# fdrmrc/fictitious_domain_AL_preconditioners

Hardware: AMD Instinct MI355X
Metric: FGMRES iterations/sec to 1e-8 residual, 3D Stokes-immersed (AL-preconditioned) (higher is better)
Workload: dtype f64

## Files before the change

fictitious_domain_al_preconditioners_amd/_abi.py:

```python
import ctypes as C

ALFD_MAX_BLOCKS = 3

OK, E_INVALID, E_HIP, E_NO_CONVERGENCE_OUTER, E_NO_CONVERGENCE_INNER, E_BREAKDOWN, E_NOT_SETUP, \
    E_COMM, E_UNSUPPORTED = range(9)
A, BT, B, CT, C_, M, MP, A2, KIMM = range(9)
NSLOTS = 9
SLOT_BY_NAME = {"A": A, "Bt": BT, "B": B, "Ct": CT, "C": C_, "M": M, "Mp": MP, "A2": A2, "K": KIMM}
INVW, MP_LUMPED_INV = 0, 1
NDIAGS = 2
AL2, AL_STOKES, AL_STOKES_DIAG, AL_ELL_IDEAL, AL_ELL_MODIFIED, RATIONAL = range(6)
CTRL_ABS, CTRL_REDUCTION, CTRL_FIXED_ITERS = range(3)
PREC_IDENTITY, PREC_JACOBI, PREC_CHEBYSHEV, PREC_MULTILEVEL = range(4)
INNER_OP_AUG, INNER_OP_A22, INNER_OP_AUG2 = range(3)
ORTH_MGS, ORTH_CGS, ORTH_CGS2 = range(3)
OUTER_FGMRES, OUTER_MINRES = range(2)
FGMRES_DEALII_96, FGMRES_DEALII_95 = range(2)
W_DIAGONAL, W_MASS_INV_SQUARED, W_MASS_INV = range(3)
INNER_THROW, INNER_ACCEPT = range(2)
T_SPMV_A, T_SPMV_OTHER, T_DOT, T_VEC = range(4)
T_NCLASSES = 4
UNIQUE_ID_BYTES = 128


class Control(C.Structure):
    _fields_ = [("kind", C.c_int32), ("max_steps", C.c_int32), ("tol", C.c_double), ("reduce", C.c_double)]

    def __init__(self, kind=CTRL_ABS, max_steps=100, tol=1e-10, reduce=0.0):
        super().__init__(kind, max_steps, tol, reduce)


class Config(C.Structure):
    _fields_ = [
        ("variant", C.c_int32), ("restart", C.c_int32), ("orthogonalization", C.c_int32),
        ("grad_div_in_A", C.c_int32),
        ("gamma", C.c_double), ("gamma_grad_div", C.c_double), ("gamma2", C.c_double),
        ("outer", Control), ("inner", Control), ("mp_inner", Control),
        ("inner_prec", C.c_int32), ("cheb_degree", C.c_int32), ("cheb_power_its", C.c_int32),
        ("on_inner_failure", C.c_int32),
        ("cheb_eig_ratio", C.c_double), ("cheb_safety", C.c_double),
        ("log_level", C.c_int32), ("outer_solver", C.c_int32),
        ("rho_bound", C.c_double), ("rational", Control),
        ("ml_smooth_degree", C.c_int32), ("ml_coarse_degree", C.c_int32),
        ("ml_smooth_ratio", C.c_double), ("ml_coarse_ratio", C.c_double),
        ("aug_assembled", C.c_int32), ("w_inverse", C.c_int32),
        ("mass", Control),
        ("fgmres_flavour", C.c_int32), ("ml_smooth_degree_coarse", C.c_int32),
        ("ml_patch_degree", C.c_int32), ("ml_coarse_direct", C.c_int32), ("ml_patch_ratio", C.c_double),
    ]


class Result(C.Structure):
    _fields_ = [
        ("status", C.c_int32), ("outer_iterations", C.c_int32),
        ("initial_residual", C.c_double), ("last_residual", C.c_double),
        ("inner_iterations", C.c_int64), ("mp_iterations", C.c_int64),
        ("inner_failures", C.c_int32), ("precond_applications", C.c_int32),
        ("solve_seconds", C.c_double), ("lambda_max", C.c_double),
        ("rational_iterations", C.c_int64), ("mass_iterations", C.c_int64),
    ]

    def as_dict(self):
        return {k: getattr(self, k) for k, _ in self._fields_}


class MatrixInfo(C.Structure):
    _fields_ = [
        ("lanes", C.c_int32), ("windowed", C.c_int32), ("value_indexed", C.c_int32), ("batch_major", C.c_int32),
        ("nnz", C.c_int64), ("window_blocks", C.c_int64), ("window_fallback_blocks", C.c_int64),
        ("value_indexed_blocks", C.c_int64), ("value_indexed_nnz", C.c_int64),
        ("dictionary_entries", C.c_int64), ("value_wide_nnz", C.c_int64),
        ("algorithmic_bytes", C.c_double), ("streamed_bytes", C.c_double),
        ("shared_nnz", C.c_int64), ("batch_major_blocks", C.c_int64), ("batch_major_wide", C.c_int64),
        ("batch_major_interior_blocks", C.c_int64),
    ]


class WindowPlanInfo(C.Structure):
    _fields_ = [
        ("windowed", C.c_int32), ("value_indexed", C.c_int32), ("row_block", C.c_int32), ("max_window", C.c_int32),
        ("blocks", C.c_int64), ("fallback_blocks", C.c_int64), ("segments", C.c_int64),
        ("value_indexed_blocks", C.c_int64), ("value_indexed_nnz", C.c_int64), ("value_wide_nnz", C.c_int64),
        ("dictionary_entries", C.c_int64), ("batches", C.c_int64), ("decode_mismatches", C.c_int64),
    ]


class StreamPlanInfo(C.Structure):
    _fields_ = [
        ("ok", C.c_int32), ("max_window", C.c_int32), ("max_rows", C.c_int32), ("max_batches", C.c_int32),
        ("blocks", C.c_int64), ("batches", C.c_int64), ("segments", C.c_int64), ("dictionary_entries", C.c_int64),
        ("stream_bytes", C.c_int64), ("decode_mismatches", C.c_int64), ("rows_covered", C.c_int64),
        ("shared_nnz", C.c_int64),
    ]


def default_config(variant=AL_STOKES) -> Config:
    c = Config()
    c.variant = variant
    c.restart = 50 if variant in (AL_ELL_IDEAL, AL_ELL_MODIFIED) else 30
    c.orthogonalization = ORTH_CGS2
    c.grad_div_in_A = 1
    c.gamma, c.gamma_grad_div, c.gamma2 = 10.0, 10.0, 1e-2
    c.outer = Control(CTRL_REDUCTION, 1000, 1e-8, 1e-12)
    c.inner = Control(CTRL_ABS, 100, 1e-2, 0.0)
# ... 34 lines not shown
```

fictitious_domain_al_preconditioners_amd/csrc/alfd.hip:

```cpp

#include <hip/hip_runtime.h>
#include <rccl/rccl.h>

#include <algorithm>
#include <atomic>
#include <chrono>
#include <cmath>
#include <cstdio>
#include <cstdlib>
#include <cstring>
#include <memory>
#include <climits>
#include <condition_variable>
#include <functional>
#include <mutex>
#include <string>
#include <thread>
#include <unordered_set>
#include <vector>

#include "alfd/alfd.h"
#include "kernels.hpp"
#include "kernels_vs.hpp"

// ... 129 lines not shown
    if (v <= c.tol) return SUCCESS;
    if (step >= c.max_steps || std::isnan(v)) return FAILURE;
    return ITERATE;
  }
};

struct TimedLaunch {
  int cls;
  hipEvent_t a, b;
};

}

using namespace alfd;

struct alfd_ctx {
  int device = 0;
  hipStream_t stream = nullptr;
  hipStream_t xstream = nullptr;
  hipEvent_t ev_x = nullptr, ev_halo = nullptr;
  int overlap_halo = -1;
  std::string err;
  int rank = 0, nranks = 1;
  ncclComm_t nccl = nullptr;
  struct alfd_local_group *local = nullptr;
  alfd_host_allgather_fn host_allgather = nullptr;
  alfd_host_alltoallv_fn host_alltoallv = nullptr;
  void *host_user = nullptr;
  std::vector<char> host_send, host_recv;
  std::vector<std::vector<int64_t>> part;
  int nblocks = 0;
  int64_t n[ALFD_MAX_BLOCKS] = {0, 0, 0};
  int64_t off[ALFD_MAX_BLOCKS + 1] = {0, 0, 0, 0};
  int64_t nmax = 0;
  int64_t diag_cap = 0;
  DevCsr mat[ALFD_NSLOTS + 1];
  double *diag[ALFD_NDIAGS] = {nullptr, nullptr};
  int64_t diag_n[ALFD_NDIAGS] = {0, 0};
  alfd_config cfg;
  bool configured = false, is_setup = false;
  double *sc = nullptr;
  double *sc_host = nullptr;
  double *partial = nullptr;
  int64_t pstride = 0;
  double *gather = nullptr;
  double *dinv_aug = nullptr, *dA = nullptr, *s_aug = nullptr;
  double *dinv_a22 = nullptr, *dinv_aug2 = nullptr;
  double lam_max[7] = {0, 0, 0, 0, 0, 0, 0};
  double *dinv_k = nullptr;
  double *dinv_m = nullptr, *m_tmp = nullptr, *m_tmp2 = nullptr;
  double *n_r = nullptr, *n_z = nullptr, *n_p = nullptr, *n_Ap = nullptr;
  double *n_sc = nullptr, *n_sc_host = nullptr, *n_partial = nullptr, *n_gather = nullptr;
  int64_t mass_its = 0;
  int n_owner = 0;
  double *gd_bx = nullptr, *gd_q = nullptr;
  int nmp_group = 16;
  int nmp_host_stepped = 0;
  HostCsr h_M, h_K;
  std::vector<int32_t> ml_agg[ALFD_MAX_LEVELS];
  std::vector<double> ml_wgt[ALFD_MAX_LEVELS];
  int64_t ml_ncoarse[ALFD_MAX_LEVELS] = {0, 0, 0, 0, 0, 0, 0, 0};
  HostCsr ml_P[ALFD_MAX_LEVELS];
  DevCsr ml_inv;
  struct Patch {
    bool on = false;
    int64_t m = 0, mpad = 0;
    DevCsr Ass, As, Ats, Cs, Cts;
    int32_t *S = nullptr;
    double *dinv = nullptr, *rS = nullptr, *zS = nullptr, *uS = nullptr, *eS = nullptr, *cd = nullptr,
           *cres = nullptr, *ctmp = nullptr, *rr = nullptr;
    double lmax = 0;
    uint8_t *tail_mask = nullptr;
    bool rep = false;
    int64_t m_loc = 0, piece = 1, lam_piece = 1;
    std::vector<int64_t> soff;
    DevCsr Cts_loc, Ctg;
    double *send = nullptr, *stage = nullptr, *lam_send = nullptr, *lam_stage = nullptr, *loc = nullptr;
  } patch;
  std::vector<MlLevel> ml;
  int ml_rep_level = -1;
  bool dots_replicated = false;
  int64_t ml_rep_threshold = 300000;
  int ml_fuse = 1;
  int ml_gpu_galerkin = 1;
  double *g_w = nullptr, *g_tlam = nullptr;
  std::vector<int64_t> ml_coff[ALFD_MAX_LEVELS];
  const int64_t *up_col_offsets = nullptr;
  bool up_local_only = false;
  DevCsr rat_mat;
  double *rt_r = nullptr, *rt_z = nullptr, *rt_p = nullptr, *rt_Ap = nullptr, *rt_x = nullptr;
  double *rt_dinv = nullptr, *rt_partial = nullptr, *rt_scb = nullptr, *rt_coef = nullptr;
  double *rt_scb_host = nullptr;
  int64_t rational_its = 0;
  int64_t wmax = 0;
  std::vector<void *> ws_allocs;
  double *w_r = nullptr, *w_z = nullptr, *w_p = nullptr, *w_Ap = nullptr;
  double *c_d = nullptr, *c_res = nullptr, *c_tmp = nullptr;
  double *t_lam = nullptr;
  double *q_tmp = nullptr, *rhs_tmp = nullptr;
  double *V = nullptr, *Z = nullptr, *xb = nullptr, *bb = nullptr, *io = nullptr;
  double *st_in = nullptr, *st_out = nullptr;
  double lambda_max = 0, lambda_min = 0;
  int64_t inner_its = 0, mp_its = 0;
  int inner_failures = 0, precond_applications = 0;
  std::vector<double> history;
  int timing = 0;
  std::vector<TimedLaunch> timed;
  double t_ms[ALFD_T_NCLASSES] = {0, 0, 0, 0};
  int64_t t_launches[ALFD_T_NCLASSES] = {0, 0, 0, 0};
  double t_bytes[ALFD_T_NCLASSES] = {0, 0, 0, 0};
  double t_fbytes[ALFD_T_NCLASSES] = {0, 0, 0, 0};
  double setup_s[ALFD_SETUP_NPHASES] = {0, 0, 0, 0, 0, 0, 0, 0};
  bool upload_since_setup = false;
  std::vector<void *> allocs;
  int spmv_stream_R = 2, spmv_stream_U = 8, spmv_nt = 0, spmv_grid_mult = 8;
  int spmv_group_R = 4, spmv_group_U = 4;
  bool vi_off = false;
  int vi_rows_R = 4, vi_rows_J = 2;
  int vi_xcd = 0;
  int vi_levels = 1;
  int vi_batched = 1;
  int win_RB_vi = 96;
  int win_vi = 1;
  int win_short_scale = 2;
  int vs_enable = 1, vs_NW = 4, vs_RB = 96, vs_xcd = 0, vs_share = 1, vs_wide = 1;
  int vs_lds_base_ok = -1;
  std::vector<int64_t> rb_ptr[ALFD_NSLOTS + 1];
  std::vector<int32_t> rb_rows[ALFD_NSLOTS + 1];
  int win_short_min_blocks = 256;
  int win_min_blocks = 256;
  int win_enable = 1, win_RB = 96, win_maxW = 4096, win_gap = 8, win_xcd = 0;
  int64_t ntot() const { return off[nblocks]; }
};

struct alfd_local_group {
  int n = 0;
  std::mutex mu;
  std::condition_variable cv;
  int arrived = 0;
  long generation = 0;
  std::vector<const void *> buf;
  std::vector<const int64_t *> off;
  void barrier() {
    std::unique_lock<std::mutex> lk(mu);
    const long g = generation;
    if (++arrived == n) {
      arrived = 0;
      ++generation;
      cv.notify_all();
    } else {
      cv.wait(lk, [&] { return generation != g; });
    }
  }
};

namespace alfd {

static int comm_allgather(alfd_ctx *ctx, const void *send, void *recv, size_t bytes) {
  if (ctx->local) {
    alfd_local_group *g = ctx->local;
    HIPC(hipStreamSynchronize(ctx->stream));
    g->buf[ctx->rank] = send;
    g->barrier();
    for (int p = 0; p < g->n; ++p)
      HIPC(hipMemcpyAsync((char *)recv + (size_t)p * bytes, g->buf[p], bytes, hipMemcpyDeviceToDevice,
                          ctx->stream));
// ... 259 lines not shown
    else ALFD_WIN(3, 0);
  } else {
    if (epi == 0) ALFD_WIN(0, 1);
    else if (epi == 1) ALFD_WIN(1, 1);
    else if (epi == 2) ALFD_WIN(2, 1);
    else ALFD_WIN(3, 1);
  }
#undef ALFD_WIN
}

template <int L, int R, int U>
static void launch_window_group(alfd_ctx *ctx, const DevCsr &m, const double *x, double *y, int epi,
                                double alpha, const double *d, double *y2) {
  const size_t lds = (size_t)m.win_maxW * sizeof(double);
#define ALFD_WING(EPI, TAG)                                                                               \
  hipLaunchKernelGGL((spmv_window_group_kernel<L, R, U, EPI, TAG>), dim3((unsigned)m.win_nblocks),       \
                     dim3(kBlock), lds, ctx->stream, m.nrows, m.win_RB, m.rp, m.col, m.lcol, m.val,        \
                     m.blk_seg_begin, m.blk_W, m.seg_col, m.seg_off, x, m.halo, m.n_local_cols, y, alpha, \
                     d, y2)
  if (m.tag == 0) {
    if (epi == 0) ALFD_WING(0, 0);
    else if (epi == 1) ALFD_WING(1, 0);
    else if (epi == 2) ALFD_WING(2, 0);
    else ALFD_WING(3, 0);
  } else {
    if (epi == 0) ALFD_WING(0, 1);
    else if (epi == 1) ALFD_WING(1, 1);
    else if (epi == 2) ALFD_WING(2, 1);
    else ALFD_WING(3, 1);
  }
#undef ALFD_WING
}

template <int L>
static bool launch_window_group_RU(alfd_ctx *ctx, const DevCsr &m, const double *x, double *y, int epi,
                                   double alpha, const double *d, double *y2) {
  const int R = ctx->spmv_group_R, U = ctx->spmv_group_U;
#define ALFD_RU(RR, UU) \
  if (R == RR && U == UU) return launch_window_group<L, RR, UU>(ctx, m, x, y, epi, alpha, d, y2), true
  ALFD_RU(4, 4); ALFD_RU(2, 4); ALFD_RU(4, 2); ALFD_RU(8, 4); ALFD_RU(8, 2);
#undef ALFD_RU
  return false;
}

static bool launch_window_RU(alfd_ctx *ctx, const DevCsr &m, const double *x, double *y, int epi,
                             double alpha, const double *d, double *y2) {
  if (m.L == 32) return launch_window_group_RU<32>(ctx, m, x, y, epi, alpha, d, y2);
  if (m.L == 16) return launch_window_group_RU<16>(ctx, m, x, y, epi, alpha, d, y2);
  if (m.L == 8) return launch_window_group_RU<8>(ctx, m, x, y, epi, alpha, d, y2);
  if (m.L != 64) return false;
  const int R = ctx->spmv_stream_R, U = ctx->spmv_stream_U;
#define ALFD_RU(RR, UU) \
  if (R == RR && U == UU) return launch_window<RR, UU>(ctx, m, x, y, epi, alpha, d, y2), true
  ALFD_RU(1, 4); ALFD_RU(2, 4); ALFD_RU(2, 8); ALFD_RU(4, 2); ALFD_RU(4, 4); ALFD_RU(4, 8); ALFD_RU(8, 4);
  ALFD_RU(1, 8); ALFD_RU(1, 16); ALFD_RU(2, 16);
#undef ALFD_RU
  return false;
}


template <int L>
static void launch_vss(alfd_ctx *ctx, const DevCsr &m, const double *x, double *y, int epi, double alpha,
                       const double *d, double *y2) {
  const DevCsr::Vs &v = m.vs;
  const size_t lds = (size_t)kVsWinOff + (size_t)v.maxW * sizeof(double);
#define ALFD_VSS(EPI, TAG)                                                                                          \
  hipLaunchKernelGGL((spmv_vss_kernel<L, EPI, TAG>), dim3((unsigned)v.nb), dim3(256), lds, ctx->stream, v.stream, \
                     v.sb, v.tab, v.cnt, v.stride, v.seg_begin, v.blkW, v.seg_col, v.seg_off, v.doff, v.dn, v.dict, \
                     x, m.halo, m.n_local_cols, y, alpha, d, y2)
  if (m.tag == 0) {
    if (epi == 0) ALFD_VSS(0, 0);
    else if (epi == 1) ALFD_VSS(1, 0);
    else if (epi == 2) ALFD_VSS(2, 0);
    else ALFD_VSS(3, 0);
  } else {
    if (epi == 0) ALFD_VSS(0, 1);
    else if (epi == 1) ALFD_VSS(1, 1);
    else if (epi == 2) ALFD_VSS(2, 1);
    else ALFD_VSS(3, 1);
  }
#undef ALFD_VSS
}

static bool launch_vs(alfd_ctx *ctx, const DevCsr &m, const double *x, double *y, int epi, double alpha,
                      const double *d, double *y2, int64_t first_block = 0, int64_t n_blocks = -1) {
  const DevCsr::Vs &v = m.vs;
  if (ctx->vs_lds_base_ok < 0) {
    uint32_t *probe = nullptr, base = 1;
    if (hipMalloc((void **)&probe, sizeof(uint32_t)) == hipSuccess) {
      hipLaunchKernelGGL(vs_lds_base_probe_kernel, dim3(1), dim3(64), 4096, ctx->stream, probe);
      hipMemcpyAsync(&base, probe, sizeof(uint32_t), hipMemcpyDeviceToHost, ctx->stream);
      hipStreamSynchronize(ctx->stream);
      hipFree(probe);
    }
    ctx->vs_lds_base_ok = base == 0 ? 1 : 0;
    if (!ctx->vs_lds_base_ok)
      std::fprintf(stderr, "[alfd] dynamic LDS does not start at offset 0 (%u): batch-major SpMV formats disabled\n", base);
  }
  if (!ctx->vs_lds_base_ok) return false;
  if (v.L == 32) return launch_vss<32>(ctx, m, x, y, epi, alpha, d, y2), true;
  if (v.L == 16) return launch_vss<16>(ctx, m, x, y, epi, alpha, d, y2), true;
  if (v.L == 8) return launch_vss<8>(ctx, m, x, y, epi, alpha, d, y2), true;
  const int NW = ctx->vs_NW;
  const size_t lds = (size_t)(v.wide ? VsFmt<1>::kWinOff : VsFmt<0>::kWinOff) + (size_t)v.maxW * sizeof(double);
  if (n_blocks < 0) n_blocks = v.nb - first_block;
  if (n_blocks <= 0) return true;
  const unsigned grid = (unsigned)n_blocks;
  const int32_t base = (int32_t)first_block;
#define ALFD_VS_ARGS \
  v.stream, v.tab, v.stride, v.hdrb, v.segx, v.seg_stride, v.dict, x, m.halo, m.n_local_cols, y, alpha, d, y2, ctx->vs_xcd, base
#define ALFD_VS(EPI, NWV)                                                                                        \
  do {                                                                                                           \
    if (v.wide)                                     \
      hipLaunchKernelGGL((spmv_vs_kernel<EPI, 0, 4, 1>), dim3(grid), dim3(256), lds, ctx->stream,     \
                         ALFD_VS_ARGS);                                                                          \
    else if (m.tag == 0)                                                                                         \
      hipLaunchKernelGGL((spmv_vs_kernel<EPI, 0, NWV>), dim3(grid), dim3(64 * NWV), lds, ctx->stream, \
                         ALFD_VS_ARGS);                                                                          \
    else                \
      hipLaunchKernelGGL((spmv_vs_kernel<EPI, 1, 4>), dim3(grid), dim3(256), lds, ctx->stream,        \
                         ALFD_VS_ARGS);                                                                          \
  } while (0)
#define ALFD_VS_E(NWV)                  \
  do {                                  \
    if (epi == 0) ALFD_VS(0, NWV);      \
    else if (epi == 1) ALFD_VS(1, NWV); \
    else if (epi == 2) ALFD_VS(2, NWV); \
    else ALFD_VS(3, NWV);               \
  } while (0)
  if (NW == 8) ALFD_VS_E(8);
  else if (NW == 2) ALFD_VS_E(2);
  else ALFD_VS_E(4);
#undef ALFD_VS_E
#undef ALFD_VS
#undef ALFD_VS_ARGS
  return true;
}

static int halo_exchange(alfd_ctx *ctx, DevCsr &m, const double *x, hipStream_t st = nullptr);
static int spmv_launch_local(alfd_ctx *ctx, DevCsr &m, const double *x, double *y, int epi, double alpha, const double *d,
                             double *y2);

static int spmv_m(alfd_ctx *ctx, DevCsr &m, int cls, const double *x, double *y, int epi, double alpha = 0.0,
                  const double *d = nullptr, double *y2 = nullptr) {
  if (!m.present) return ctx->err = "matrix not set", ALFD_E_NOT_SETUP;
  const bool exchange = ctx->nranks > 1 && !m.rep && (ctx->local || ctx->host_alltoallv || m.n_halo > 0 || m.send_off.back() > 0);
  const bool overlap = exchange && (ctx->overlap_halo > 0 || (ctx->overlap_halo < 0 && (ctx->local || ctx->host_alltoallv))) && ctx->xstream && m.vs.on && m.vs.L == 64 && ctx->vs_enable && !ctx->vi_off &&
                       m.vs.nb_interior > 0 && !m.sparse && m.n_list > 0;
  if (overlap) {
    Timer tm(ctx, cls, m.algorithmic_bytes(), m.streamed_bytes(true, true));
    HIPC(hipEventRecord(ctx->ev_x, ctx->stream));
    if (!launch_vs(ctx, m, x, y, epi, alpha, d, y2, 0, m.vs.nb_interior)) return ctx->err = "batch-major launch failed", ALFD_E_HIP;
    HIPC(hipStreamWaitEvent(ctx->xstream, ctx->ev_x, 0));
    RC(halo_exchange(ctx, m, x, ctx->xstream));
    HIPC(hipEventRecord(ctx->ev_halo, ctx->xstream));
    HIPC(hipStreamWaitEvent(ctx->stream, ctx->ev_halo, 0));
    launch_vs(ctx, m, x, y, epi, alpha, d, y2, m.vs.nb_interior, m.vs.nb - m.vs.nb_interior);
    HIPC(hipGetLastError());
    return ALFD_OK;
  }
  if (exchange) RC(halo_exchange(ctx, m, x));
  if (m.sparse && epi != 1) {
    HIPC(hipMemsetAsync(y, 0, m.nrows * sizeof(double), ctx->stream));
    if (epi == 3) HIPC(hipMemsetAsync(y2, 0, m.nrows * sizeof(double), ctx->stream));
  }
  if (m.n_list == 0) return ALFD_OK;
  Timer tm(ctx, cls, m.algorithmic_bytes(), m.streamed_bytes(!ctx->vi_off, ctx->vs_enable != 0 && !ctx->vi_off));
  return spmv_launch_local(ctx, m, x, y, epi, alpha, d, y2);
}

static int spmv_launch_local(alfd_ctx *ctx, DevCsr &m, const double *x, double *y, int epi, double alpha, const double *d,
                             double *y2) {
  if (m.vs.on && ctx->vs_enable && !ctx->vi_off && launch_vs(ctx, m, x, y, epi, alpha, d, y2)) {
    HIPC(hipGetLastError());
    return ALFD_OK;
  }
  if (m.win && launch_window_RU(ctx, m, x, y, epi, alpha, d, y2)) {
    HIPC(hipGetLastError());
    return ALFD_OK;
  }
  if (m.L == 64 && !m.sparse && ctx->spmv_stream_R > 0) {
    const bool ok = ctx->spmv_nt ? launch_stream_RU<true>(ctx, m, x, y, epi, alpha, d, y2)
// ... 2569 lines not shown
  out.ncols = n_cols_c;
  out.rp.assign(1, 0);
  out.col.clear();
  out.val.clear();
  for (int t = 0; t < T; ++t) {
    for (int64_t c : t_cnt[t]) out.rp.push_back(out.rp.back() + c);
    out.col.insert(out.col.end(), t_col[t].begin(), t_col[t].end());
    out.val.insert(out.val.end(), t_val[t].begin(), t_val[t].end());
  }
}

static int upload_matrix(alfd_ctx *ctx, int slot, int64_t nrows, int64_t ncols, const int64_t *rp,
                         const int32_t *col, const double *val);
static int upload_level(alfd_ctx *ctx, DevCsr &dst, const HostCsr &h) {
  static const int32_t no_col = 0;
  static const double no_val = 0;
  RC(upload_matrix(ctx, kScratchSlot, h.nrows, h.ncols, h.rp.data(), h.col.empty() ? &no_col : h.col.data(),
                   h.val.empty() ? &no_val : h.val.data()));
  csr_free(dst);
  dst = std::move(ctx->mat[kScratchSlot]);
  ctx->mat[kScratchSlot] = DevCsr();
  dst.tag = 1;
  return ALFD_OK;
}

struct AugOp {
  DevCsr *A = nullptr, *C = nullptr, *Ct = nullptr;
  int clsA = ALFD_T_SPMV_OTHER;
  const double *w = nullptr;
  double *tlam = nullptr;
  const uint8_t *mask = nullptr;
  int64_t npad = 0;
  const double *dinv = nullptr;
  double *cd = nullptr, *cres = nullptr, *ctmp = nullptr;
  double lmax = 0;
};

struct LevelView {
  AugOp op;
  double *r = nullptr, *z = nullptr, *t = nullptr;
  DevCsr *R = nullptr, *P = nullptr;
  double *rc = nullptr, *zc = nullptr;
};

static LevelView level_view(alfd_ctx *ctx, int l) {
  MlLevel &L = ctx->ml[l];
  const bool rep = ctx->ml_rep_level >= 0 && l >= ctx->ml_rep_level;
  LevelView V;
  AugOp &F = V.op;
  F.A = rep ? &L.gA : l == 0 ? &ctx->mat[ALFD_A] : &L.A;
  F.C = rep ? &L.gC : l == 0 ? &ctx->mat[ALFD_C] : &L.C;
  F.Ct = rep ? &L.gCt : l == 0 ? &ctx->mat[ALFD_CT] : &L.Ct;
  F.clsA = l == 0 ? ALFD_T_SPMV_A : ALFD_T_SPMV_OTHER;
  F.w = rep ? ctx->g_w : ctx->diag[ALFD_INVW];
  F.tlam = rep ? ctx->g_tlam : ctx->t_lam;
  F.mask = L.tail_mask;
  F.npad = rep ? L.gnpad : L.npad;
  F.dinv = rep ? L.gdinv : L.dinv;
  F.cd = rep ? L.gcd : L.cd, F.cres = rep ? L.gcres : L.cres, F.ctmp = rep ? L.gctmp : L.ctmp;
  F.lmax = L.lmax;
  V.r = rep ? L.gr : L.r, V.z = rep ? L.gz : L.z, V.t = rep ? L.gt : L.t;
  if (l + 1 < (int)ctx->ml.size()) {
    MlLevel &N = ctx->ml[l + 1];
    V.R = rep ? &N.gR : &N.R, V.P = rep ? &N.gP : &N.P;
    V.rc = rep ? N.gr : N.r, V.zc = rep ? N.gz : N.z;
  }
  return V;
}

static AugOp patch_aug(alfd_ctx *ctx) {
  alfd_ctx::Patch &Q = ctx->patch;
  AugOp F;
  F.A = &Q.Ass, F.C = &Q.Cs, F.Ct = &Q.Cts;
  F.w = Q.rep ? ctx->g_w : ctx->diag[ALFD_INVW];
  F.tlam = Q.rep ? ctx->g_tlam : ctx->t_lam;
  F.mask = Q.tail_mask;
  F.npad = Q.mpad;
  F.dinv = Q.dinv;
  F.cd = Q.cd, F.cres = Q.cres, F.ctmp = Q.ctmp;
  F.lmax = Q.lmax;
  return F;
}

static int fused_AC(alfd_ctx *ctx, const AugOp &F, const double *x, double *y) {
  RC(spmv_m(ctx, *F.A, F.clsA, x, y, 0));
  return spmv_m(ctx, *F.C, ALFD_T_SPMV_OTHER, x, F.tlam, 2, 0.0, F.w);
}

static int aug_apply(alfd_ctx *ctx, const AugOp &F, const double *x, double *y) {
  if (ctx->cfg.aug_assembled) return spmv_m(ctx, *F.A, F.clsA, x, y, 0);
  RC(fused_AC(ctx, F, x, y));
  return spmv_m(ctx, *F.Ct, ALFD_T_SPMV_OTHER, F.tlam, y, 1, ctx->cfg.gamma);
}


static bool plain_form(const alfd_ctx *ctx, const DevCsr &m) {
  return m.present && !m.vs.on && !m.win && !(m.L == 64 && !m.sparse && ctx->spmv_stream_R > 0);
}

static bool fused_ok(const alfd_ctx *ctx, const AugOp &F) {
  return ctx->ml_fuse && ctx->nranks == 1 && !ctx->cfg.aug_assembled && !gd_nested(ctx) &&
         ctx->cfg.w_inverse == ALFD_W_DIAGONAL && F.mask && F.A->present && F.C->present && plain_form(ctx, *F.Ct);
}

static int aug_tail(alfd_ctx *ctx, const AugOp &F, int mode, const AugTailArgs &p, double vec_bytes) {
  const DevCsr &m = *F.Ct;
  const int nb_rows = m.n_list > 0 ? grid_for_rows(m.n_list, m.L) : 0;
  const unsigned grid = (unsigned)nb_rows + (unsigned)(F.npad / kChunk);
  if (grid == 0) return ALFD_OK;
  Timer tm(ctx, ALFD_T_SPMV_OTHER, m.algorithmic_bytes() + vec_bytes * (double)F.npad,
           m.streamed_bytes(false) + vec_bytes * (double)F.npad);
#define ALFD_TAIL(LL, MM)                                                                                         \
  hipLaunchKernelGGL((aug_tail_kernel<LL, MM>), dim3(grid), dim3(kBlock), 0, ctx->stream, m.n_list, m.rp, m.col,  \
                     m.val, m.sparse ? m.rows : (const int32_t *)nullptr, F.tlam, nb_rows, F.mask, p)
#define ALFD_TAIL_L(LL)                                      \
  switch (mode) {                                            \
    case TAIL_STEP: ALFD_TAIL(LL, TAIL_STEP); break;         \
    case TAIL_LAST: ALFD_TAIL(LL, TAIL_LAST); break;         \
    case TAIL_LAST_ADD: ALFD_TAIL(LL, TAIL_LAST_ADD); break; \
    case TAIL_RES: ALFD_TAIL(LL, TAIL_RES); break;           \
    case TAIL_RES_INIT: ALFD_TAIL(LL, TAIL_RES_INIT); break; \
    default: ALFD_TAIL(LL, TAIL_RES_INIT_ADD); break;        \
  }
  switch (m.L) {
    case 4: ALFD_TAIL_L(4) break;
    case 8: ALFD_TAIL_L(8) break;
    case 16: ALFD_TAIL_L(16) break;
    case 32: ALFD_TAIL_L(32) break;
    default: ALFD_TAIL_L(64) break;
  }
#undef ALFD_TAIL_L
#undef ALFD_TAIL
  HIPC(hipGetLastError());
  return ALFD_OK;
}

static int cheb_fused(alfd_ctx *ctx, const AugOp &F, int degree, double ratio, const double *r, double *z, double *zout,
                      bool have_init) {
  ChebCoef k(F.lmax, ratio);
  if (!have_init) VEC_LAUNCH(cheb_init_z_kernel, F.npad, 24, 1.0 / k.theta, F.dinv, r, z);
  for (int j = 1; j < degree; ++j) {
    RC(fused_AC(ctx, F, j == 1 ? z : F.cd, F.ctmp));
    AugTailArgs p;
    k.step(p.c1, p.c2);
    p.gamma = ctx->cfg.gamma;
    p.dinv = F.dinv, p.y = F.ctmp, p.rin = j == 1 ? r : F.cres, p.din = j == 1 ? z : F.cd;
    p.res = F.cres, p.d = F.cd, p.z = z, p.zout = zout;
    const bool last = j == degree - 1;
    RC(aug_tail(ctx, F, !last ? TAIL_STEP : zout ? TAIL_LAST_ADD : TAIL_LAST, p, last && zout ? 88.0 : 64.0));
  }
  HIPC(hipGetLastError());
  return ALFD_OK;
}

static int aug_cheb(alfd_ctx *ctx, const AugOp &F, int degree, double ratio, const double *r, double *z) {
  if (fused_ok(ctx, F)) return cheb_fused(ctx, F, degree, ratio, r, z, nullptr, false);
  return cheb_sweep(ctx, F.npad, F.dinv, F.lmax, ratio, degree, F.cd, F.cres, F.ctmp, r, z,
                    [&](const double *x, double *y) { return aug_apply(ctx, F, x, y); });
}

static int fused_residual(alfd_ctx *ctx, const AugOp &F, const double *r, double *t) {
  AugTailArgs p;
  p.gamma = ctx->cfg.gamma, p.y = t, p.rin = r, p.res = t;
  return aug_tail(ctx, F, TAIL_RES, p, 24.0);
}

static int fused_correct(alfd_ctx *ctx, const AugOp &F, int degree, double ratio, const double *r, double *t, double *zc,
                         double *zout) {
  AugTailArgs p;
// ... 56 lines not shown
  }
  if (fuse) {
    RC(fused_AC(ctx, F, z, L.t));
    RC(fused_correct(ctx, F, sdeg, c.ml_smooth_ratio, r, L.t, L.r, z));
    return ALFD_OK;
  }
  RC(aug_apply(ctx, F, z, L.t));
  VEC_LAUNCH(sub_from_kernel, F.npad, 24, r, L.t);
  RC(aug_cheb(ctx, F, sdeg, c.ml_smooth_ratio, L.t, L.r));
  VEC_LAUNCH(axpy_kernel, F.npad, 24, (const double *)nullptr, 0, 1.0, L.r, z);
  HIPC(hipGetLastError());
  return ALFD_OK;
}

static int allgather_pieces(alfd_ctx *ctx, const double *mine, const std::vector<int64_t> &offs, int64_t piece, double *send,
                            double *stage, double *whole) {
  const int64_t n_me = offs[ctx->rank + 1] - offs[ctx->rank];
  if (n_me > 0) HIPC(hipMemcpyAsync(send, mine, n_me * sizeof(double), hipMemcpyDeviceToDevice, ctx->stream));
  RC(comm_allgather(ctx, send, stage, (size_t)piece * sizeof(double)));
  for (int p = 0; p < ctx->nranks; ++p) {
    const int64_t np = offs[p + 1] - offs[p];
    if (np > 0)
      HIPC(hipMemcpyAsync(whole + offs[p], stage + (int64_t)p * piece, np * sizeof(double), hipMemcpyDeviceToDevice, ctx->stream));
  }
  return ALFD_OK;
}

static int ml_apply_rep(alfd_ctx *ctx, const double *r, double *z) {
  alfd_ctx::Patch &Q = ctx->patch;
  const int64_t n0p = pad_chunk(ctx->n[0]);
  const unsigned gm = (unsigned)std::max<int64_t>(1, (Q.m_loc + 255) / 256);
  const bool pen = !ctx->cfg.aug_assembled;
  const int last = ctx->nblocks - 1;
  const int64_t s0 = Q.soff[ctx->rank];
  const AugOp F = patch_aug(ctx);
  const int pdeg = ctx->cfg.ml_patch_degree;
  const double pratio = ctx->cfg.ml_patch_ratio;
  if (Q.m_loc > 0) hipLaunchKernelGGL(gather_kernel, dim3(gm), dim3(256), 0, ctx->stream, Q.m_loc, Q.S, r, Q.loc);
  RC(allgather_pieces(ctx, Q.loc, Q.soff, Q.piece, Q.send, Q.stage, Q.rS));
  RC(aug_cheb(ctx, F, pdeg, pratio, Q.rS, Q.zS));
  VEC_LAUNCH(scale_copy_kernel, n0p, 16, 1.0, r, Q.rr);
  RC(spmv_m(ctx, Q.Ats, ALFD_T_SPMV_OTHER, Q.zS, Q.rr, 1, -1.0));
  if (pen) {
    RC(spmv_m(ctx, Q.Cs, ALFD_T_SPMV_OTHER, Q.zS, ctx->g_tlam, 2, 0.0, ctx->g_w));
    RC(spmv_m(ctx, Q.Ctg, ALFD_T_SPMV_OTHER, ctx->g_tlam, Q.rr, 1, -ctx->cfg.gamma));
  }
  RC(ml_cycle(ctx, 0, Q.rr, z));
  if (Q.m_loc > 0) hipLaunchKernelGGL(scatter_add_kernel, dim3(gm), dim3(256), 0, ctx->stream, Q.m_loc, Q.S, Q.zS + s0, z);
  RC(spmv_m(ctx, Q.As, ALFD_T_SPMV_OTHER, z, Q.loc, 0));
  if (pen) {
    RC(spmv(ctx, ALFD_C, z, ctx->t_lam, 2, 0.0, ctx->diag[ALFD_INVW]));
    RC(allgather_pieces(ctx, ctx->t_lam, ctx->part[last], Q.lam_piece, Q.lam_send, Q.lam_stage, ctx->g_tlam));
    RC(spmv_m(ctx, Q.Cts_loc, ALFD_T_SPMV_OTHER, ctx->g_tlam, Q.loc, 1, ctx->cfg.gamma));
  }
  RC(allgather_pieces(ctx, Q.loc, Q.soff, Q.piece, Q.send, Q.stage, Q.uS));
  VEC_LAUNCH(sub_from_kernel, Q.mpad, 24, Q.rS, Q.uS);
  RC(aug_cheb(ctx, F, pdeg, pratio, Q.uS, Q.eS));
  if (Q.m_loc > 0) hipLaunchKernelGGL(scatter_add_kernel, dim3(gm), dim3(256), 0, ctx->stream, Q.m_loc, Q.S, Q.eS + s0, z);
  HIPC(hipGetLastError());
  return ALFD_OK;
}

static int ml_apply(alfd_ctx *ctx, const double *r, double *z) {
  alfd_ctx::Patch &Q = ctx->patch;
  if (!Q.on) return ml_cycle(ctx, 0, r, z);
  if (Q.rep) return ml_apply_rep(ctx, r, z);
  const int64_t n0p = pad_chunk(ctx->n[0]);
  const unsigned gm = (unsigned)((Q.m + 255) / 256);
  const bool pen = !ctx->cfg.aug_assembled;
  const double *w = ctx->diag[ALFD_INVW];
  const AugOp F = patch_aug(ctx);
  const int pdeg = ctx->cfg.ml_patch_degree;
  const double pratio = ctx->cfg.ml_patch_ratio;
  hipLaunchKernelGGL(gather_kernel, dim3(gm), dim3(256), 0, ctx->stream, Q.m, Q.S, r, Q.rS);
  RC(aug_cheb(ctx, F, pdeg, pratio, Q.rS, Q.zS));
  VEC_LAUNCH(scale_copy_kernel, n0p, 16, 1.0, r, Q.rr);
  RC(spmv_m(ctx, Q.Ats, ALFD_T_SPMV_OTHER, Q.zS, Q.rr, 1, -1.0));
  if (pen) {
    RC(spmv_m(ctx, Q.Cs, ALFD_T_SPMV_OTHER, Q.zS, ctx->t_lam, 2, 0.0, w));
    RC(spmv(ctx, ALFD_CT, ctx->t_lam, Q.rr, 1, -ctx->cfg.gamma));
  }
  RC(ml_cycle(ctx, 0, Q.rr, z));
  hipLaunchKernelGGL(scatter_add_kernel, dim3(gm), dim3(256), 0, ctx->stream, Q.m, Q.S, Q.zS, z);
  RC(spmv_m(ctx, Q.As, ALFD_T_SPMV_OTHER, z, Q.uS, 0));
  if (fused_ok(ctx, F)) {
    RC(spmv(ctx, ALFD_C, z, ctx->t_lam, 2, 0.0, w));
    RC(fused_correct(ctx, F, pdeg, pratio, Q.rS, Q.uS, Q.eS, nullptr));
  } else {
    if (pen) {
      RC(spmv(ctx, ALFD_C, z, ctx->t_lam, 2, 0.0, w));
      RC(spmv_m(ctx, Q.Cts, ALFD_T_SPMV_OTHER, ctx->t_lam, Q.uS, 1, ctx->cfg.gamma));
    }
    VEC_LAUNCH(sub_from_kernel, Q.mpad, 24, Q.rS, Q.uS);
    RC(aug_cheb(ctx, F, pdeg, pratio, Q.uS, Q.eS));
  }
  hipLaunchKernelGGL(scatter_add_kernel, dim3(gm), dim3(256), 0, ctx->stream, Q.m, Q.S, Q.eS, z);
  HIPC(hipGetLastError());
  return ALFD_OK;
}

static void spgemm_host(const HostCsr &A, const HostCsr &Pm, HostCsr &out) {
  const int64_t nrows = A.nrows, nc = Pm.ncols;
  const int T = (int)std::max<int64_t>(1, std::min<int64_t>(std::min(16u, std::max(1u, std::thread::hardware_concurrency())),
                                                           (nrows + 4095) / 4096));
  std::vector<std::vector<int32_t>> t_cnt(T), t_col(T);
  std::vector<std::vector<double>> t_val(T);
  std::vector<std::thread> th;
  for (int t = 0; t < T; ++t)
    th.emplace_back([&, t]() {
      const int64_t i0 = nrows * t / T, i1 = nrows * (t + 1) / T;
      std::vector<int64_t> stamp(nc, -1);
      std::vector<double> acc(nc, 0.0);
      std::vector<int32_t> touched;
      t_cnt[t].reserve(i1 - i0);
      for (int64_t i = i0; i < i1; ++i) {
        touched.clear();
        for (int64_t k = A.rp[i]; k < A.rp[i + 1]; ++k) {
          const double a = A.val[k];
          const int64_t j = A.col[k];
          for (int64_t e = Pm.rp[j]; e < Pm.rp[j + 1]; ++e) {
            const int32_t J = Pm.col[e];
            if (stamp[J] != i) {
              stamp[J] = i;
              acc[J] = std::fma(a, Pm.val[e], 0.0);
              touched.push_back(J);
            } else {
              acc[J] = std::fma(a, Pm.val[e], acc[J]);
            }
          }
        }
        std::sort(touched.begin(), touched.end());
        t_cnt[t].push_back((int32_t)touched.size());
        for (int32_t J : touched) {
          t_col[t].push_back(J);
          t_val[t].push_back(acc[J]);
        }
      }
    });
  for (auto &x : th) x.join();
  out.nrows = nrows;
  out.ncols = nc;
  out.rp.assign(1, 0);
  out.rp.reserve(nrows + 1);
  int64_t total = 0;
  for (int t = 0; t < T; ++t) total += (int64_t)t_col[t].size();
  out.col.clear();
  out.val.clear();
  out.col.reserve(total);
  out.val.reserve(total);
  for (int t = 0; t < T; ++t) {
    for (int32_t c : t_cnt[t]) out.rp.push_back(out.rp.back() + c);
    out.col.insert(out.col.end(), t_col[t].begin(), t_col[t].end());
    out.val.insert(out.val.end(), t_val[t].begin(), t_val[t].end());
    std::vector<int32_t>().swap(t_col[t]);
    std::vector<double>().swap(t_val[t]);
  }
}

static void extract_host(const HostCsr &A, const std::vector<int32_t> &rows, const int32_t *colmap, int64_t ncols,
                         bool full_rows, HostCsr &out) {
  out.nrows = full_rows ? A.nrows : (int64_t)rows.size();
  out.ncols = ncols;
  out.rp.assign(out.nrows + 1, 0);
  out.col.clear();
  out.val.clear();
  int64_t next = 0;
  for (size_t q = 0; q < rows.size(); ++q) {
    const int64_t i = rows[q], orow = full_rows ? i : (int64_t)q;
    for (; next <= orow; ++next) out.rp[next] = (int64_t)out.col.size();
    for (int64_t k = A.rp[i]; k < A.rp[i + 1]; ++k) {
      const int32_t c = colmap ? colmap[A.col[k]] : A.col[k];
      if (c < 0) continue;
      out.col.push_back(c);
      out.val.push_back(A.val[k]);
    }
// ... 1646 lines not shown
    HIPC(hipMemcpyAsync(blocks[b], dev + ctx->off[b], ctx->n[b] * sizeof(double), hipMemcpyDeviceToHost,
                        ctx->stream));
  HIPC(hipStreamSynchronize(ctx->stream));
  return ALFD_OK;
}

static void reset_stats(alfd_ctx *ctx) {
  ctx->inner_its = ctx->mp_its = 0;
  ctx->inner_failures = ctx->precond_applications = 0;
  ctx->rational_its = 0;
  ctx->mass_its = 0;
}
static void fill_result(alfd_ctx *ctx, alfd_result *res, int status) {
  res->status = status;
  res->inner_iterations = ctx->inner_its;
  res->mp_iterations = ctx->mp_its;
  res->inner_failures = ctx->inner_failures;
  res->precond_applications = ctx->precond_applications;
  res->lambda_max = ctx->lambda_max;
  res->rational_iterations = ctx->rational_its;
  res->mass_iterations = ctx->mass_its;
}

}

#define CHECK_CTX()                       \
  if (!ctx) return ALFD_E_INVALID;        \
  if (hipSetDevice(ctx->device) != hipSuccess) return ctx->err = "hipSetDevice failed", ALFD_E_HIP
#define CHECK_SETUP() \
  if (!ctx->is_setup) return ctx->err = "alfd_setup not called", ALFD_E_NOT_SETUP

extern "C" {

int alfd_abi_version(void) { return ALFD_ABI_VERSION; }

const char *alfd_strerror(int s) {
  switch (s) {
    case ALFD_OK: return "ok";
    case ALFD_E_INVALID: return "invalid argument";
    case ALFD_E_HIP: return "HIP runtime error";
    case ALFD_E_NO_CONVERGENCE_OUTER: return "FGMRES: no convergence (SolverControl::NoConvergence)";
    case ALFD_E_NO_CONVERGENCE_INNER: return "inner CG: no convergence (SolverControl::NoConvergence)";
    case ALFD_E_BREAKDOWN: return "breakdown (NaN residual)";
    case ALFD_E_NOT_SETUP: return "context not set up";
    case ALFD_E_COMM: return "RCCL error";
    case ALFD_E_UNSUPPORTED: return "not implemented";
    default: return "unknown status";
  }
}

const char *alfd_last_error(alfd_ctx_t ctx) { return ctx ? ctx->err.c_str() : "null context"; }

int alfd_create(alfd_ctx_t *out, int device_id) {
  if (!out) return ALFD_E_INVALID;
  *out = nullptr;
  int ndev = 0;
  if (hipGetDeviceCount(&ndev) != hipSuccess || ndev <= 0 || device_id < 0 || device_id >= ndev)
    return ALFD_E_HIP;
  if (hipSetDevice(device_id) != hipSuccess) return ALFD_E_HIP;
  alfd_ctx *ctx = new alfd_ctx;
  ctx->device = device_id;
  if (hipStreamCreateWithFlags(&ctx->xstream, hipStreamNonBlocking) != hipSuccess ||
      hipEventCreateWithFlags(&ctx->ev_x, hipEventDisableTiming) != hipSuccess ||
      hipEventCreateWithFlags(&ctx->ev_halo, hipEventDisableTiming) != hipSuccess)
    ctx->xstream = nullptr;
  if (const char *e = std::getenv("ALFD_SPMV_OVERLAP_HALO")) ctx->overlap_halo = std::atoi(e);
  if (hipStreamCreateWithFlags(&ctx->stream, hipStreamNonBlocking) != hipSuccess) {
    delete ctx;
    return ALFD_E_HIP;
  }
  alfd_default_config(&ctx->cfg, ALFD_AL_STOKES);
  if (const char *e = std::getenv("ALFD_SPMV_STREAM_R")) ctx->spmv_stream_R = std::atoi(e);
  if (const char *e = std::getenv("ALFD_SPMV_STREAM_U")) ctx->spmv_stream_U = std::atoi(e);
  if (const char *e = std::getenv("ALFD_SPMV_NT")) ctx->spmv_nt = std::atoi(e);
  if (const char *e = std::getenv("ALFD_SPMV_GRID")) ctx->spmv_grid_mult = std::max(1, std::atoi(e));
  if (const char *e = std::getenv("ALFD_SPMV_WINDOW")) ctx->win_enable = std::atoi(e);
  if (const char *e = std::getenv("ALFD_SPMV_WINDOW_RB")) ctx->win_RB = std::max(4, std::atoi(e));
  if (const char *e = std::getenv("ALFD_SPMV_WINDOW_MIN_BLOCKS")) ctx->win_min_blocks = std::max(1, std::atoi(e));
  if (const char *e = std::getenv("ALFD_SPMV_WINDOW_SHORT_MIN_BLOCKS")) ctx->win_short_min_blocks = std::max(1, std::atoi(e));
  if (const char *e = std::getenv("ALFD_SPMV_WINDOW_MAXW")) ctx->win_maxW = std::min(16384, std::max(256, std::atoi(e)));
  if (const char *e = std::getenv("ALFD_ML_REPLICATE")) ctx->ml_rep_threshold = std::atoll(e);
  if (const char *e = std::getenv("ALFD_ML_GPU_GALERKIN")) ctx->ml_gpu_galerkin = std::atoi(e);
  if (const char *e = std::getenv("ALFD_ML_FUSE")) ctx->ml_fuse = std::atoi(e) != 0;
  if (const char *e = std::getenv("ALFD_SPMV_VI_LEVELS")) ctx->vi_levels = std::atoi(e);
  if (const char *e = std::getenv("ALFD_SPMV_BATCH_MAJOR")) ctx->vs_enable = std::atoi(e);
  if (const char *e = std::getenv("ALFD_SPMV_BATCH_MAJOR_ROWS")) ctx->vs_RB = std::max(4, std::min(kVsMaxRows, std::atoi(e)));
  if (const char *e = std::getenv("ALFD_SPMV_VI_XCD")) ctx->vi_xcd = std::atoi(e);
  if (const char *e = std::getenv("ALFD_SPMV_VI_BATCHED")) ctx->vi_batched = std::atoi(e);
  if (const char *e = std::getenv("ALFD_SPMV_WINDOW_RB_VI")) ctx->win_RB_vi = std::atoi(e);
  if (const char *e = std::getenv("ALFD_SPMV_VI_R")) ctx->vi_rows_R = std::atoi(e);
  if (const char *e = std::getenv("ALFD_SPMV_VI_J")) ctx->vi_rows_J = std::atoi(e);
  if (const char *e = std::getenv("ALFD_SPMV_VALUE_INDEX")) ctx->win_vi = std::atoi(e);
  if (const char *e = std::getenv("ALFD_SPMV_GROUP_R")) ctx->spmv_group_R = std::atoi(e);
  if (const char *e = std::getenv("ALFD_SPMV_GROUP_U")) ctx->spmv_group_U = std::atoi(e);
  if (const char *e = std::getenv("ALFD_SPMV_WINDOW_SHORT")) ctx->win_short_scale = std::max(0, std::atoi(e));
  if (const char *e = std::getenv("ALFD_SPMV_WINDOW_GAP")) ctx->win_gap = std::max(1, std::atoi(e));
  if (const char *e = std::getenv("ALFD_SPMV_WINDOW_XCD")) ctx->win_xcd = std::atoi(e);
  *out = ctx;
  return ALFD_OK;
}

int alfd_destroy(alfd_ctx_t ctx) {
  if (!ctx) return ALFD_E_INVALID;
  hipSetDevice(ctx->device);
  hipStreamSynchronize(ctx->stream);
  flush_timers(ctx);
  free_levels(ctx);
  csr_free(ctx->rat_mat);
  for (DevCsr &m : ctx->mat) csr_free(m);
  for (void *p : ctx->ws_allocs) hipFree(p);
  for (void *p : ctx->allocs) hipFree(p);
  if (ctx->sc_host) hipHostFree(ctx->sc_host);
  if (ctx->n_sc_host) hipHostFree(ctx->n_sc_host);
  if (ctx->rt_scb_host) hipHostFree(ctx->rt_scb_host);
  if (ctx->nccl) ncclCommDestroy(ctx->nccl);
  if (ctx->xstream) hipStreamDestroy(ctx->xstream);
  if (ctx->ev_x) hipEventDestroy(ctx->ev_x);
  if (ctx->ev_halo) hipEventDestroy(ctx->ev_halo);
  hipStreamDestroy(ctx->stream);
  delete ctx;
  return ALFD_OK;
}

int alfd_comm_unique_id(void *id_out, size_t bytes) {
  static_assert(sizeof(ncclUniqueId) <= ALFD_UNIQUE_ID_BYTES, "unique id size");
  if (!id_out || bytes < sizeof(ncclUniqueId)) return ALFD_E_INVALID;
  ncclUniqueId id;
  if (ncclGetUniqueId(&id) != ncclSuccess) return ALFD_E_COMM;
  std::memset(id_out, 0, bytes);
  std::memcpy(id_out, &id, sizeof(id));
  return ALFD_OK;
}

int alfd_comm_init(alfd_ctx_t ctx, int rank, int nranks, const void *id, size_t bytes) {
  CHECK_CTX();
  if (nranks < 1 || rank < 0 || rank >= nranks) return ALFD_E_INVALID;
  ctx->rank = rank;
  ctx->nranks = nranks;
  if (nranks == 1) return ALFD_OK;
  if (!id || bytes < sizeof(ncclUniqueId)) return ALFD_E_INVALID;
  ncclUniqueId uid;
  std::memcpy(&uid, id, sizeof(uid));
  if (ncclCommInitRank(&ctx->nccl, nranks, uid, rank) != ncclSuccess)
    return ctx->err = "ncclCommInitRank failed", ALFD_E_COMM;
  if (rank == 0) {
    int v = 0;
    if (ncclGetVersion(&v) == ncclSuccess) std::fprintf(stderr, "[alfd] RCCL version %d, %d ranks\n", v, nranks);
  }
  return ALFD_OK;
}

int alfd_local_group_create(int nranks, alfd_local_group **out) {
  if (!out || nranks < 1) return ALFD_E_INVALID;
  alfd_local_group *g = new alfd_local_group;
  g->n = nranks;
  g->buf.assign(nranks, nullptr);
  g->off.assign(nranks, nullptr);
  *out = g;
  return ALFD_OK;
}

int alfd_local_group_destroy(alfd_local_group *g) {
  if (!g) return ALFD_E_INVALID;
  delete g;
  return ALFD_OK;
}
// ... 1092 lines not shown
}

int alfd_host_permute_csr(int64_t nrows, const int64_t *rp, const int32_t *col, const double *val,
                          const int64_t *row_new_to_old, const int64_t *col_old_to_new, int64_t *orp, int32_t *ocol,
                          double *oval) {
  if (nrows < 0 || !rp || !orp || (rp[nrows] > 0 && (!col || !val || !ocol || !oval))) return ALFD_E_INVALID;
  orp[0] = 0;
  for (int64_t r = 0; r < nrows; ++r) {
    const int64_t src = row_new_to_old ? row_new_to_old[r] : r;
    if (src < 0 || src >= nrows) return ALFD_E_INVALID;
    orp[r + 1] = orp[r] + (rp[src + 1] - rp[src]);
  }
  if (orp[nrows] != rp[nrows]) return ALFD_E_INVALID;
  const int T = (int)std::max<int64_t>(1, std::min<int64_t>(std::min(16u, std::max(1u, std::thread::hardware_concurrency())),
                                                           (nrows + 8191) / 8192));
  std::vector<std::thread> th;
  for (int t = 0; t < T; ++t)
    th.emplace_back([&, t]() {
      std::vector<std::pair<int32_t, double>> row;
      for (int64_t r = nrows * t / T; r < nrows * (t + 1) / T; ++r) {
        const int64_t src = row_new_to_old ? row_new_to_old[r] : r;
        const int64_t k0 = rp[src], len = rp[src + 1] - k0, o0 = orp[r];
        if (!col_old_to_new) {
          for (int64_t k = 0; k < len; ++k) ocol[o0 + k] = col[k0 + k], oval[o0 + k] = val[k0 + k];
          continue;
        }
        row.resize(len);
        for (int64_t k = 0; k < len; ++k) row[k] = {(int32_t)col_old_to_new[col[k0 + k]], val[k0 + k]};
        std::sort(row.begin(), row.end(), [](const auto &x, const auto &y) { return x.first < y.first; });
        for (int64_t k = 0; k < len; ++k) ocol[o0 + k] = row[k].first, oval[o0 + k] = row[k].second;
      }
    });
  for (auto &x : th) x.join();
  return ALFD_OK;
}

int alfd_get_device_memory(alfd_ctx_t ctx, int64_t *free_bytes, int64_t *total_bytes) {
  CHECK_CTX();
  size_t f = 0, t = 0;
  HIPC(hipMemGetInfo(&f, &t));
  if (free_bytes) *free_bytes = (int64_t)f;
  if (total_bytes) *total_bytes = (int64_t)t;
  return ALFD_OK;
}

int alfd_set_tunable(alfd_ctx_t ctx, const char *name, int value) {
  if (!ctx || !name) return ALFD_E_INVALID;
  if (std::strcmp(name, "value_index") == 0) {
    ctx->vi_off = value == 0;
    if (value == 0) RC(ensure_window_plans(ctx));
    return ALFD_OK;
  }
  if (std::strcmp(name, "batch_major") == 0) {
    ctx->vs_enable = value != 0;
    if (value == 0) RC(ensure_window_plans(ctx));
    return ALFD_OK;
  }
  if (std::strcmp(name, "batch_major_share") == 0) {
    ctx->vs_share = value != 0;
    return ALFD_OK;
  }
  if (std::strcmp(name, "batch_major_wide") == 0) {
    ctx->vs_wide = value != 0;
    return ALFD_OK;
  }
  if (std::strcmp(name, "batch_major_waves") == 0) {
    if (value != 2 && value != 4 && value != 8) return ctx->err = "batch_major_waves: 2, 4 or 8", ALFD_E_INVALID;
    ctx->vs_NW = value;
    return ALFD_OK;
  }
  if (std::strcmp(name, "batch_major_rows") == 0) {
    if (value < 4 || value > kVsMaxRows) return ctx->err = "batch_major_rows: 4..250", ALFD_E_INVALID;
    ctx->vs_RB = value;
    return ALFD_OK;
  }
  if (std::strcmp(name, "batch_major_xcd") == 0) {
    ctx->vs_xcd = value != 0;
    return ALFD_OK;
  }
  if (std::strcmp(name, "ml_fuse") == 0) {
    ctx->ml_fuse = value != 0;
    return ALFD_OK;
  }
  if (std::strcmp(name, "nested_mp_group") == 0) {
    if (value < 1 || value > 1000) return ctx->err = "nested_mp_group: 1..1000", ALFD_E_INVALID;
    ctx->nmp_group = value;
    return ALFD_OK;
  }
  if (std::strcmp(name, "nested_mp_host_stepped") == 0) {
    ctx->nmp_host_stepped = value != 0;
    return ALFD_OK;
  }
  return ctx->err = std::string("unknown tunable ") + name, ALFD_E_INVALID;
}

int alfd_set_row_blocks(alfd_ctx_t ctx, int slot, int64_t n_blocks, const int64_t *block_ptr, const int32_t *rows) {
  if (!ctx || slot < 0 || slot >= ALFD_NSLOTS) return ALFD_E_INVALID;
  ctx->rb_ptr[slot].clear();
  ctx->rb_rows[slot].clear();
  if (n_blocks <= 0 || !block_ptr || !rows) return ALFD_OK;
  if (block_ptr[0] != 0) return ctx->err = "alfd_set_row_blocks: block_ptr[0] must be 0", ALFD_E_INVALID;
  for (int64_t b = 0; b < n_blocks; ++b)
    if (block_ptr[b + 1] < block_ptr[b]) return ctx->err = "alfd_set_row_blocks: block_ptr must be monotone", ALFD_E_INVALID;
  if (block_ptr[n_blocks] > 2147483000LL) return ctx->err = "alfd_set_row_blocks: more than 2^31 rows", ALFD_E_INVALID;
  ctx->rb_ptr[slot].assign(block_ptr, block_ptr + n_blocks + 1);
  ctx->rb_rows[slot].assign(rows, rows + block_ptr[n_blocks]);
  return ALFD_OK;
}

int alfd_enable_timing(alfd_ctx_t ctx, int on) {
  if (!ctx) return ALFD_E_INVALID;
  ctx->timing = on < 0 ? 0 : on;
  for (int i = 0; i < ALFD_T_NCLASSES; ++i) ctx->t_ms[i] = 0, ctx->t_launches[i] = 0, ctx->t_bytes[i] = 0, ctx->t_fbytes[i] = 0;
  return ALFD_OK;
}
int alfd_get_timing_streamed(alfd_ctx_t ctx, double *streamed_bytes) {
  if (!ctx || !streamed_bytes) return ALFD_E_INVALID;
  for (int i = 0; i < ALFD_T_NCLASSES; ++i) streamed_bytes[i] = ctx->t_fbytes[i];
  return ALFD_OK;
}
int alfd_get_setup_seconds(alfd_ctx_t ctx, double *seconds) {
  if (!ctx || !seconds) return ALFD_E_INVALID;
  for (int i = 0; i < ALFD_SETUP_NPHASES; ++i) seconds[i] = ctx->setup_s[i];
  return ALFD_OK;
}

int alfd_get_timing(alfd_ctx_t ctx, double *ms, int64_t *launches, double *bytes) {
  if (!ctx) return ALFD_E_INVALID;
  flush_timers(ctx);
  for (int i = 0; i < ALFD_T_NCLASSES; ++i) {
    if (ms) ms[i] = ctx->t_ms[i];
    if (launches) launches[i] = ctx->t_launches[i];
    if (bytes) bytes[i] = ctx->t_bytes[i];
  }
  return ALFD_OK;
}

}
```

fictitious_domain_al_preconditioners_amd/csrc/kernels.hpp:

```cpp
#pragma once
#include <hip/hip_runtime.h>
#include <stdint.h>

namespace alfd {

constexpr int kBlock = 256;
constexpr int64_t kChunk = 4096;
constexpr int kMaxBasis = 64;

__device__ __forceinline__ double dpp_xor_mov(double v, int which) {
  int lo = __double2loint(v), hi = __double2hiint(v), rl, rh;
  if (which == 8) {
    rl = __builtin_amdgcn_update_dpp(0, lo, 0x128, 0xf, 0xf, true);
    rh = __builtin_amdgcn_update_dpp(0, hi, 0x128, 0xf, 0xf, true);
  } else if (which == 4) {
    rl = __builtin_amdgcn_update_dpp(0, lo, 0x104, 0xf, 0x5, false);
    rl = __builtin_amdgcn_update_dpp(rl, lo, 0x114, 0xf, 0xa, false);
    rh = __builtin_amdgcn_update_dpp(0, hi, 0x104, 0xf, 0x5, false);
    rh = __builtin_amdgcn_update_dpp(rh, hi, 0x114, 0xf, 0xa, false);
  } else if (which == 2) {
    rl = __builtin_amdgcn_update_dpp(0, lo, 0x4E, 0xf, 0xf, true);
    rh = __builtin_amdgcn_update_dpp(0, hi, 0x4E, 0xf, 0xf, true);
  } else {
    rl = __builtin_amdgcn_update_dpp(0, lo, 0xB1, 0xf, 0xf, true);
// ... 42 lines not shown
__device__ __forceinline__ double row16_tree(double v) {
  v = v + dpp_xor_mov(v, 8);
  v = v + dpp_shl<4>(v);
  v = v + dpp_shl<2>(v);
  v = v + dpp_shl<1>(v);
  return v;
}
__device__ __forceinline__ double reduce_rows4(double a0, double a1, double a2, double a3) {
  swap32(a0, a1);
  double p = a0 + a1;
  swap32(a2, a3);
  double q = a2 + a3;
  swap16(p, q);
  return row16_tree(p + q);
}
__device__ __forceinline__ double reduce_rows8(double a0, double a1, double a2, double a3, double a4, double a5,
                                               double a6, double a7, int lane) {
  swap32(a0, a1);
  double p01 = a0 + a1;
  swap32(a2, a3);
  double p23 = a2 + a3;
  swap32(a4, a5);
  double p45 = a4 + a5;
  swap32(a6, a7);
  double p67 = a6 + a7;
  swap16(p01, p23);
  double u = p01 + p23;
  swap16(p45, p67);
  double w = p45 + p67;
  u = u + dpp_xor_mov(u, 8);
  w = w + dpp_xor_mov(w, 8);
  double x = (lane & 8) ? w : u;
  x = x + dpp_shl<4>(x);
  x = x + dpp_shl<2>(x);
  x = x + dpp_shl<1>(x);
  return x;
}

template <int N>
__device__ __forceinline__ double dpp_shr(double v) {
  const int lo = __double2loint(v), hi = __double2hiint(v);
  const int rl = __builtin_amdgcn_update_dpp(0, lo, 0x110 + N, 0xf, 0xf, true);
  const int rh = __builtin_amdgcn_update_dpp(0, hi, 0x110 + N, 0xf, 0xf, true);
  return __hiloint2double(rh, rl);
}
__device__ __forceinline__ double reduce_rows16(double (&a)[16], int lane) {
  double p[8], u[4];
#pragma unroll
  for (int j = 0; j < 8; ++j) {
    swap32(a[2 * j], a[2 * j + 1]);
    p[j] = a[2 * j] + a[2 * j + 1];
  }
#pragma unroll
  for (int j = 0; j < 4; ++j) {
    swap16(p[2 * j], p[2 * j + 1]);
    u[j] = p[2 * j] + p[2 * j + 1];
    u[j] = u[j] + dpp_xor_mov(u[j], 8);
  }
  const bool h = (lane & 8) != 0;
  double x0 = h ? u[1] : u[0], x1 = h ? u[3] : u[2];
  x0 = x0 + dpp_shl<4>(x0);
  x1 = x1 + dpp_shr<4>(x1);
  double z = (lane & 4) ? x1 : x0;
  z = z + dpp_shl<2>(z);
  z = z + dpp_shl<1>(z);
  return z;
}

__device__ __forceinline__ double reduce_rows2(double a0, double a1) {
  swap32(a0, a1);
  double p = a0 + a1, q = p;
  swap16(p, q);
  return row16_tree(p + q);
}

__device__ __forceinline__ double block_reduce_256(double v, double *lds4) {
  v = group_reduce<64>(v);
  const int wave = threadIdx.x >> 6;
  if ((threadIdx.x & 63) == 0) lds4[wave] = v;
  __syncthreads();
  return (lds4[0] + lds4[1]) + (lds4[2] + lds4[3]);
}

template <int L, int EPI, bool SPARSE>
__global__ __launch_bounds__(kBlock) void spmv_kernel(int64_t nrows, const int64_t *__restrict__ rp,
                                                      const int32_t *__restrict__ col,
                                                      const double *__restrict__ val,
                                                      const int32_t *__restrict__ rows,
                                                      const double *__restrict__ x,
                                                      const double *__restrict__ x_halo, int32_t n_local,
                                                      double *__restrict__ y, double alpha,
                                                      const double *__restrict__ d,
                                                      double *__restrict__ y2) {
  constexpr int RPB = kBlock / L;
  const int lane = threadIdx.x % L;
  const int sub = threadIdx.x / L;
  const int64_t ngroups = (nrows + RPB - 1) / RPB;
  for (int64_t g = blockIdx.x; g < ngroups; g += gridDim.x) {
    const int64_t r = g * RPB + sub;
    if (r < nrows) {
      const int64_t k0 = rp[r], k1 = rp[r + 1];
      double acc = 0.0;
      for (int64_t k = k0 + lane; k < k1; k += L) {
        const int32_t c = col[k];
        const double xv = (c < n_local) ? x[c] : x_halo[c - n_local];
        acc = fma(val[k], xv, acc);
      }
      acc = group_reduce<L>(acc);
      if (lane == 0) {
        const int64_t ro = SPARSE ? (int64_t)rows[r] : r;
        if (EPI == 0)
          y[ro] = acc;
        else if (EPI == 1)
          y[ro] = fma(alpha, acc, y[ro]);
        else if (EPI == 2)
          y[ro] = d[ro] * acc;
        else {
          y[ro] = acc;
          y2[ro] = d[ro] * acc;
        }
      }
    }
  }
}

template <int R, int U, int EPI, bool NT>
__global__ __launch_bounds__(kBlock) void spmv_stream_kernel(
    int64_t nrows, const int64_t *__restrict__ rp, const int32_t *__restrict__ col,
    const double *__restrict__ val, const double *__restrict__ x, const double *__restrict__ x_halo,
    int32_t n_local, double *__restrict__ y, double alpha, const double *__restrict__ d,
    double *__restrict__ y2) {
  const int lane = threadIdx.x & 63;
  const int wave = __builtin_amdgcn_readfirstlane(threadIdx.x >> 6);
  const int64_t nbatches = (nrows + R - 1) / R;
  for (int64_t b = (int64_t)blockIdx.x * 4 + wave; b < nbatches; b += (int64_t)gridDim.x * 4) {
    const int64_t r0 = b * R;
    int64_t kb[R + 1];
#pragma unroll
    for (int i = 0; i <= R; ++i) kb[i] = rp[r0 + i < nrows ? r0 + i : nrows];
    const int64_t k_begin = kb[0];
    const int32_t n_batch = (int32_t)(kb[R] - k_begin);
    int32_t rel[R + 1];
#pragma unroll
    for (int i = 0; i <= R; ++i) rel[i] = (int32_t)(kb[i] - k_begin);
    double acc[R];
#pragma unroll
    for (int i = 0; i < R; ++i) acc[i] = 0.0;
    const int32_t *cb = col + k_begin;
    const double *vb = val + k_begin;
    for (int32_t base = 0; base < n_batch; base += 64 * U) {
      int32_t c[U];
      double v[U], xv[U];
#pragma unroll
      for (int u = 0; u < U; ++u) {
        const int32_t o = base + 64 * u + lane;
        if (o < n_batch) {
          c[u] = NT ? __builtin_nontemporal_load(cb + o) : cb[o];
          v[u] = NT ? __builtin_nontemporal_load(vb + o) : vb[o];
        } else {
          c[u] = -1;
          v[u] = 0.0;
        }
      }
#pragma unroll
      for (int u = 0; u < U; ++u) {
        xv[u] = 0.0;
        if (c[u] >= 0) xv[u] = (c[u] < n_local) ? x[c[u]] : x_halo[c[u] - n_local];
      }
#pragma unroll
      for (int u = 0; u < U; ++u) {
        const int32_t o = base + 64 * u + lane;
        if (c[u] >= 0) {
#pragma unroll
          for (int i = 0; i < R; ++i)
            if (o >= rel[i] && o < rel[i + 1]) acc[i] = fma(v[u], xv[u], acc[i]);
        }
      }
    }
#pragma unroll
    for (int i = 0; i < R; ++i) {
      const int64_t r = r0 + i;
      if (r < nrows) {
        const int dsh = rel[i] & 63;
        double s = __shfl(acc[i], (lane + dsh) & 63, 64);
        s = group_reduce<64>(s);
        if (lane == 0) {
          if (EPI == 0)
            y[r] = s;
          else if (EPI == 1)
            y[r] = fma(alpha, s, y[r]);
          else if (EPI == 2)
            y[r] = d[r] * s;
          else {
            y[r] = s;
            y2[r] = d[r] * s;
          }
        }
      }
    }
  }
}

template <int R, int U, int EPI, int TAG = 0>
__global__ __launch_bounds__(kBlock) void spmv_window_kernel(
    int64_t nrows, int32_t RB, const int64_t *__restrict__ rp, const int32_t *__restrict__ col,
    const uint16_t *__restrict__ lcol, const double *__restrict__ val,
    const int32_t *__restrict__ blk_seg_begin, const int32_t *__restrict__ blk_W,
    const int32_t *__restrict__ seg_col, const int32_t *__restrict__ seg_off,
    const double *__restrict__ x, const double *__restrict__ x_halo, int32_t n_local,
    double *__restrict__ y, double alpha, const double *__restrict__ d, double *__restrict__ y2,
    int xcd_remap) {
  extern __shared__ double xs[];
  const int lane = threadIdx.x & 63;
  const int wave = __builtin_amdgcn_readfirstlane(threadIdx.x >> 6);
  int64_t b = blockIdx.x;
  if (xcd_remap) {
    const int64_t nwg = gridDim.x, q = nwg / 8, rm = nwg % 8, xcd = b % 8, idx = b / 8;
    b = (xcd < rm ? xcd * (q + 1) : rm * (q + 1) + (xcd - rm) * q) + idx;
  }
  const int32_t W = blk_W[b];
  if (W >= 0) {
    const int32_t s0 = blk_seg_begin[b], s1 = blk_seg_begin[b + 1];
    for (int32_t s = s0 + wave; s < s1; s += 4) {
      const int32_t c0 = seg_col[s], o0 = seg_off[s];
      const int32_t len = ((s + 1 < s1) ? seg_off[s + 1] : W) - o0;
      for (int32_t i = lane; i < len; i += 64) {
        const int32_t c = c0 + i;
        xs[o0 + i] = (c < n_local) ? x[c] : x_halo[c - n_local];
      }
    }
    __syncthreads();
  }
  const int64_t row_begin = b * RB;
  const int64_t row_end = (row_begin + RB < nrows) ? row_begin + RB : nrows;
  for (int64_t r0 = row_begin + (int64_t)wave * R; r0 < row_end; r0 += 4 * R) {
    int64_t kb[R + 1];
#pragma unroll
    for (int i = 0; i <= R; ++i) kb[i] = rp[r0 + i < row_end ? r0 + i : row_end];
    const int64_t k_begin = kb[0];
    const int32_t n_batch = (int32_t)(kb[R] - k_begin);
    int32_t rel[R + 1];
#pragma unroll
    for (int i = 0; i <= R; ++i) rel[i] = (int32_t)(kb[i] - k_begin);
    double acc[R];
#pragma unroll
    for (int i = 0; i < R; ++i) acc[i] = 0.0;
    const double *vb = val + k_begin;
    if (W >= 0) {
      const uint16_t *cb = lcol + k_begin;
      for (int32_t base = 0; base < n_batch; base += 64 * U) {
        int32_t c[U];
        double v[U], xv[U];
#pragma unroll
        for (int u = 0; u < U; ++u) {
          const int32_t o = base + 64 * u + lane;
          if (o < n_batch) {
            c[u] = cb[o];
            v[u] = vb[o];
          } else {
            c[u] = -1;
            v[u] = 0.0;
          }
        }
#pragma unroll
        for (int u = 0; u < U; ++u) xv[u] = c[u] >= 0 ? xs[c[u]] : 0.0;
#pragma unroll
        for (int u = 0; u < U; ++u) {
          const int32_t o = base + 64 * u + lane;
          if (c[u] >= 0) {
#pragma unroll
            for (int i = 0; i < R; ++i)
              if (o >= rel[i] && o < rel[i + 1]) acc[i] = fma(v[u], xv[u], acc[i]);
          }
        }
      }
    } else {
      const int32_t *cb = col + k_begin;
      for (int32_t base = 0; base < n_batch; base += 64 * U) {
#pragma unroll
        for (int u = 0; u < U; ++u) {
          const int32_t o = base + 64 * u + lane;
          if (o < n_batch) {
            const int32_t c = cb[o];
// ... 1404 lines not shown
```

fictitious_domain_al_preconditioners_amd/csrc/kernels_vs.hpp:

```cpp
#pragma once

namespace alfd {

constexpr int kVsMaxDict = 512;
constexpr int kVsDictOff = 0;
constexpr int kVsWinOff = kVsMaxDict * 8;
constexpr int kVsMaxRows = 250;
template <int WD>
struct VsFmt {
  static constexpr uint32_t kColMask = WD ? 0x3ff8u : 0x7ff8u;
  static constexpr int kDictShift = WD ? 11 : 12;
  static constexpr uint32_t kDictMask = WD ? 0x1ff8u : 0xff8u;
  static constexpr int kWinOff = WD ? 8192 : 4096;
  static constexpr int kCodeShift = WD ? 14 : 15;
  static constexpr int kMaxDict = WD ? 1024 : 512;
  static constexpr int kMaxSlots = WD ? 2048 : 4096;
};
constexpr int kVsMaxLen = 384;

__device__ __forceinline__ uint32_t vs_off(uint32_t d) { return d & 0xfffffu; }
__device__ __forceinline__ int32_t vs_len(uint32_t d) { return (int32_t)((d >> 20) & 0x1ffu); }
__device__ __forceinline__ int vs_cls(uint32_t d) { return (int)((d >> 29) & 7u); }

__device__ __forceinline__ double vs_lds_f64(uint32_t byte_off) {
// ... 13 lines not shown
__device__ __forceinline__ void vs_batch(const int32_t (&rem)[4], int32_t maxrem, int lane,
                                         const uint8_t *__restrict__ fb, const char *sm, double (&acc)[4]) {
  VsWord3 w[NCH];
#pragma unroll
  for (int j = 0; j < NCH - 1; ++j) w[j] = *(const VsWord3 *)(fb + 768 * j + 12u * (uint32_t)lane);
  w[NCH - 1] = *(const VsWord3 *)(fb + 768 * (NCH - 1) + 12u * (uint32_t)(lane < maxrem ? lane : maxrem - 1));
#pragma unroll
  for (int j = 0; j < NCH; ++j) {
    double xv[4], v[4];
    const uint32_t f[4] = {w[j].x, __builtin_amdgcn_alignbit(w[j].y, w[j].x, 24),
                           __builtin_amdgcn_alignbit(w[j].z, w[j].y, 16), w[j].z >> 8};
#pragma unroll
    for (int i = 0; i < 4; ++i) {
      xv[i] = vs_lds_f64(VsFmt<WD>::kWinOff + (f[i] & VsFmt<WD>::kColMask));
      v[i] = vs_lds_f64(kVsDictOff + ((f[i] >> VsFmt<WD>::kDictShift) & VsFmt<WD>::kDictMask));
    }
#pragma unroll
    for (int i = 0; i < 4; ++i) asm volatile("" : "+v"(xv[i]), "+v"(v[i]));
#pragma unroll
    for (int i = 0; i < 4; ++i) {
      if (j == NCH - 1) {
        if (lane < rem[i]) acc[i] = fma(v[i], xv[i], acc[i]);
      } else {
        acc[i] = fma(v[i], xv[i], acc[i]);
      }
    }
  }
}

__device__ __forceinline__ void vs_shared_fetch(uint32_t d0, const uint8_t *__restrict__ sbase, int lane, uint32_t (&w)[6]) {
  const int cls = vs_cls(d0);
  const uint8_t *fb = sbase + 16u * (size_t)vs_off(d0);
  const int32_t rem = vs_len(d0) - 64 * (cls - 1);
  uint32_t l4 = 4u * (uint32_t)lane, r4 = 4u * (uint32_t)(lane < rem ? lane : rem - 1);
  asm volatile("" : "+v"(l4), "+v"(r4));
  w[0] = *(const uint32_t *)(fb + 256 * (cls - 1) + r4);
#pragma unroll
  for (int j = 0; j < 5; ++j)
    if (j < cls - 1) w[1 + j] = *(const uint32_t *)(fb + 256 * j + l4);
}

template <int NCH, int R, int WD>
__device__ __forceinline__ void vs_shared(int32_t rem, const int32_t (&sh)[R], int lane, const uint32_t (&w)[6],
                                          double (&acc)[R]) {
#pragma unroll
  for (int j = 0; j < NCH; ++j) {
    const uint32_t wj = j == NCH - 1 ? w[0] : w[1 + (j < 5 ? j : 0)];
    const uint32_t lc = wj & VsFmt<WD>::kColMask;
    double v = vs_lds_f64(kVsDictOff + ((wj >> VsFmt<WD>::kDictShift) & VsFmt<WD>::kDictMask));
    constexpr int G = R > 8 ? 4 : R;
#pragma unroll
    for (int g = 0; g < R; g += G) {
      double xv[G];
#pragma unroll
      for (int i = 0; i < G; ++i) xv[i] = vs_lds_f64(VsFmt<WD>::kWinOff + (uint32_t)((int32_t)lc + sh[g + i]));
#pragma unroll
      for (int i = 0; i < G; ++i) asm volatile("" : "+v"(xv[i]));
      if (g == 0) asm volatile("" : "+v"(v));
      if (j == NCH - 1) {
        if (lane < rem) {
          asm volatile("");
#pragma unroll
          for (int i = 0; i < G; ++i) acc[g + i] = fma(v, xv[i], acc[g + i]);
        }
      } else {
#pragma unroll
        for (int i = 0; i < G; ++i) acc[g + i] = fma(v, xv[i], acc[g + i]);
      }
      if (R > 8) {
#pragma unroll
        for (int i = 0; i < G; ++i) asm volatile("" : "+v"(acc[g + i]));
      }
    }
  }
}

template <int EPI, int TAG, int NW, int WD = 0>
__global__ __launch_bounds__(64 * NW) __attribute__((amdgpu_waves_per_eu(8, 8))) void spmv_vs_kernel(
    const uint8_t *__restrict__ stream, const uint64_t *__restrict__ tab, int32_t stride,
    const int32_t *__restrict__ hdrb, const int32_t *__restrict__ segx, int32_t seg_stride,
    const double *__restrict__ dict, const double *__restrict__ x, const double *__restrict__ x_halo,
    int32_t n_local, double *__restrict__ y, double alpha, const double *__restrict__ d, double *__restrict__ y2,
    int xcd_remap, int32_t block_base) {
  extern __shared__ double xs[];
  char *sm = (char *)xs;
  double *ds = (double *)(sm + kVsDictOff);
  double *xw = (double *)(sm + VsFmt<WD>::kWinOff);
  const int lane = threadIdx.x & 63;
  const int wave = __builtin_amdgcn_readfirstlane(threadIdx.x >> 6);
  int64_t b = blockIdx.x;
  if (xcd_remap) {
    const int64_t nwg = gridDim.x, q = nwg / 8, rm = nwg % 8, xcd = b % 8, idx = b / 8;
    b = (xcd < rm ? xcd * (q + 1) : rm * (q + 1) + (xcd - rm) * q) + idx;
  }
  b += block_base;
  const int32_t *hb = hdrb + 8 * b;
  const int32_t nbatch = hb[0], W = hb[1], nseg = hb[2], nd = hb[3], doff = hb[4];
  const uint8_t *sbase = stream + (int64_t)(((uint64_t)(uint32_t)hb[6] << 32) | (uint64_t)(uint32_t)hb[5]);
  const int32_t *sx = segx + 2 * b * (int64_t)seg_stride;
  const uint32_t *tb = (const uint32_t *)(tab + (int64_t)b * stride * 16);
  const int hl = lane & 31;
  auto hdr_at = [&](int32_t q) {
    uint32_t h4 = 4u * (uint32_t)hl;
    asm volatile("" : "+v"(h4));
    return *(const uint32_t *)((const char *)(tb + 32 * (int64_t)q) + h4);
  };
  auto hdr_load = [&](int32_t q) {
    return hdr_at(q < nbatch ? q : (nbatch > 0 ? nbatch - 1 : 0));
  };
  auto hdr = [](uint32_t hv, int k) { return (uint32_t)__builtin_amdgcn_readlane((int)hv, k); };
  uint32_t hv1 = hdr_at(wave);
  uint32_t hv2 = hdr_at(wave + NW);
  uint32_t w[6];
  {
    constexpr int U = 4;
    auto stage = [&](int32_t s) {
      int32_t c0[U], o0[U], sl[U];
      double v[U];
#pragma unroll
      for (int u = 0; u < U; ++u) {
        const int32_t q = s + u;
        c0[u] = sx[2 * q];
        o0[u] = sx[2 * q + 1];
        const int32_t on = sx[2 * q + 3];
        sl[u] = q < nseg ? ((q + 1 < nseg ? on : W) - o0[u]) : 0;
      }
#pragma unroll
      for (int u = 0; u < U; ++u) {
        const int32_t c = c0[u] + (lane < sl[u] ? lane : 0);
        v[u] = (c < n_local) ? x[c] : x_halo[c - n_local];
      }
#pragma unroll
      for (int u = 0; u < U; ++u)
        if (lane < sl[u]) xw[o0[u] + lane] = v[u];
    };
    for (int t = threadIdx.x; t < nd; t += 64 * NW) ds[t] = dict[doff + t];
    if (wave < nbatch && (int32_t)hdr(hv1, 1) < 0) vs_shared_fetch(hdr(hv1, 0), sbase, lane, w);
    stage(wave * U);
    for (int32_t s = (wave + NW) * U; s < nseg; s += NW * U) stage(s);
  }
  __syncthreads();
  const int q16 = lane >> 4;
  const int rsel = 4 * (2 * ((((q16 & 1) << 1) | (q16 >> 1)) + 4 * ((lane >> 3) & 1) + 8 * ((lane >> 2) & 1)) + 1);
  auto store = [&](double s, int32_t r, bool mine) {
    if (mine && r >= 0) {
      if (EPI == 0)
        y[r] = s;
      else if (EPI == 1)
        y[r] = fma(alpha, s, y[r]);
      else if (EPI == 2)
        y[r] = d[r] * s;
      else {
        y[r] = s;
        y2[r] = d[r] * s;
      }
    }
  };
  for (int32_t bi = wave; bi < nbatch; bi += NW) {
    uint32_t lo[16];
#pragma unroll
    for (int i = 0; i < 16; ++i) lo[i] = hdr(hv1, 2 * i);
    const bool shared = (int32_t)hdr(hv1, 1) < 0;
    const bool sixteen = shared && (int32_t)hdr(hv1, 17) >= 0;
    const bool eight = shared && !sixteen && (int32_t)hdr(hv1, 9) >= 0;
    const uint32_t eb = vs_off(lo[0]);
    const int cls = vs_cls(lo[0]);
    const int32_t full = cls > 0 ? 64 * (cls - 1) : 0;
    const uint8_t *fb = sbase + 16u * (size_t)eb;
    double sres;
    int mstep;
    uint32_t n0, n1;
    if (sixteen) {
      const int32_t rem = vs_len(lo[0]) - full;
      int32_t sh[16];
      sh[0] = 0;
#pragma unroll
      for (int i = 1; i < 16; ++i) sh[i] = (int32_t)lo[i];
      double acc[16] = {0.0, 0.0, 0.0, 0.0, 0.0, 0.0, 0.0, 0.0, 0.0, 0.0, 0.0, 0.0, 0.0, 0.0, 0.0, 0.0};
      switch (cls) {
        case 1: vs_shared<1, 16, WD>(rem, sh, lane, w, acc); break;
        case 2: vs_shared<2, 16, WD>(rem, sh, lane, w, acc); break;
        case 3: vs_shared<3, 16, WD>(rem, sh, lane, w, acc); break;
        case 4: vs_shared<4, 16, WD>(rem, sh, lane, w, acc); break;
        case 5: vs_shared<5, 16, WD>(rem, sh, lane, w, acc); break;
        default: vs_shared<6, 16, WD>(rem, sh, lane, w, acc); break;
      }
      sres = reduce_rows16(acc, lane);
      mstep = 4;
    } else if (eight) {
      const int32_t rem = vs_len(lo[0]) - full;
      int32_t sh[8];
      sh[0] = 0;
#pragma unroll
      for (int i = 1; i < 8; ++i) sh[i] = (int32_t)lo[i];
      double acc[8] = {0.0, 0.0, 0.0, 0.0, 0.0, 0.0, 0.0, 0.0};
      switch (cls) {
        case 1: vs_shared<1, 8, WD>(rem, sh, lane, w, acc); break;
        case 2: vs_shared<2, 8, WD>(rem, sh, lane, w, acc); break;
        case 3: vs_shared<3, 8, WD>(rem, sh, lane, w, acc); break;
        case 4: vs_shared<4, 8, WD>(rem, sh, lane, w, acc); break;
        case 5: vs_shared<5, 8, WD>(rem, sh, lane, w, acc); break;
        default: vs_shared<6, 8, WD>(rem, sh, lane, w, acc); break;
      }
      sres = reduce_rows8(acc[0], acc[1], acc[2], acc[3], acc[4], acc[5], acc[6], acc[7], lane);
      mstep = 8;
    } else if (shared) {
      double acc[4] = {0.0, 0.0, 0.0, 0.0};
      const int32_t rem = vs_len(lo[0]) - full;
      const int32_t sh[4] = {0, (int32_t)lo[1], (int32_t)lo[2], (int32_t)lo[3]};
      switch (cls) {
        case 1: vs_shared<1, 4, WD>(rem, sh, lane, w, acc); break;
        case 2: vs_shared<2, 4, WD>(rem, sh, lane, w, acc); break;
        case 3: vs_shared<3, 4, WD>(rem, sh, lane, w, acc); break;
        case 4: vs_shared<4, 4, WD>(rem, sh, lane, w, acc); break;
        case 5: vs_shared<5, 4, WD>(rem, sh, lane, w, acc); break;
        default: vs_shared<6, 4, WD>(rem, sh, lane, w, acc); break;
      }
      sres = reduce_rows4(acc[0], acc[1], acc[2], acc[3]);
      mstep = 16;
    } else {
      double acc[4] = {0.0, 0.0, 0.0, 0.0};
      int32_t rem[4], maxrem = 1;
#pragma unroll
      for (int i = 0; i < 4; ++i) {
        rem[i] = vs_len(lo[i]) - full;
        maxrem = rem[i] > maxrem ? rem[i] : maxrem;
      }
      switch (cls) {
        case 1: vs_batch<1, WD>(rem, maxrem, lane, fb, sm, acc); break;
        case 2: vs_batch<2, WD>(rem, maxrem, lane, fb, sm, acc); break;
        case 3: vs_batch<3, WD>(rem, maxrem, lane, fb, sm, acc); break;
        case 4: vs_batch<4, WD>(rem, maxrem, lane, fb, sm, acc); break;
        case 5: vs_batch<5, WD>(rem, maxrem, lane, fb, sm, acc); break;
        case 6: vs_batch<6, WD>(rem, maxrem, lane, fb, sm, acc); break;
        default: break;
      }
      n0 = hdr(hv2, 0);
      n1 = hdr(hv2, 1);
      store(reduce_rows4(acc[0], acc[1], acc[2], acc[3]), (int32_t)__builtin_amdgcn_ds_bpermute(rsel, (int)hv1), (lane & 15) == 0);
      mstep = 0;
    }
    int32_t rid = -1;
    if (mstep) {
      rid = (int32_t)((uint32_t)__builtin_amdgcn_ds_bpermute(rsel, (int)hv1) &
                      (lane < 8 ? 0x7fffffffu : 0xffffffffu));
      n0 = hdr(hv2, 0);
      n1 = hdr(hv2, 1);
    }
    hv1 = hv2;
    if (bi + NW < nbatch && (int32_t)n1 < 0) vs_shared_fetch(n0, sbase, lane, w);
    hv2 = hdr_load(bi + 2 * NW);
    if (mstep) store(sres, rid, (lane & (mstep - 1)) == 0);
  }
}

template <int L, int EPI, int TAG>
__global__ __launch_bounds__(256) __attribute__((amdgpu_waves_per_eu(8, 8))) void spmv_vss_kernel(
    const uint8_t *__restrict__ stream, const int64_t *__restrict__ sb, const uint64_t *__restrict__ tab,
    const int32_t *__restrict__ cnt, int32_t stride, const int32_t *__restrict__ blk_seg_begin,
    const int32_t *__restrict__ blk_W, const int32_t *__restrict__ seg_col, const int32_t *__restrict__ seg_off,
    const int32_t *__restrict__ blk_dict_off, const int32_t *__restrict__ blk_dict_n,
    const double *__restrict__ dict, const double *__restrict__ x, const double *__restrict__ x_halo,
    int32_t n_local, double *__restrict__ y, double alpha, const double *__restrict__ d, double *__restrict__ y2) {
  extern __shared__ double xs[];
  constexpr int G = 64 / L, W64 = 1 + 4 * G, NW = 4;
  char *sm = (char *)xs;
  double *ds = (double *)(sm + kVsDictOff);
  double *xw = (double *)(sm + kVsWinOff);
  const int lane = threadIdx.x & 63;
  const int wave = __builtin_amdgcn_readfirstlane(threadIdx.x >> 6);
  const int l = lane & (L - 1), g = lane / L;
  const int64_t b = blockIdx.x;
  const int32_t nbatch = cnt[b];
  const uint8_t *sbase = stream + sb[b];
  {
    const int32_t nd = blk_dict_n[b];
    for (int t = threadIdx.x; t < nd; t += 64 * NW) ds[t] = dict[blk_dict_off[b] + t];
    const int32_t W = blk_W[b];
    const int32_t s0 = blk_seg_begin[b], s1 = blk_seg_begin[b + 1];
    constexpr int U = 4;
    for (int32_t s = s0 + wave * U; s < s1; s += NW * U) {
      int32_t c0[U], o0[U], sl[U];
      double v[U];
#pragma unroll
      for (int u = 0; u < U; ++u) {
        const int32_t q = s + u < s1 ? s + u : s1 - 1;
        c0[u] = seg_col[q];
        o0[u] = seg_off[q];
        sl[u] = ((q + 1 < s1) ? seg_off[q + 1] : W) - o0[u];
      }
#pragma unroll
      for (int u = 0; u < U; ++u) {
        const int32_t c = c0[u] + (lane < sl[u] ? lane : 0);
        v[u] = (c < n_local) ? x[c] : x_halo[c - n_local];
      }
#pragma unroll
      for (int u = 0; u < U; ++u)
        if (lane < sl[u]) xw[o0[u] + lane] = v[u];
    }
  }
  __syncthreads();
  const uint64_t *dsc = tab + ((int64_t)b * stride + wave) * W64;
  auto load_batch = [&](const uint64_t *dp, uint64_t hh, uint64_t (&e)[4], uint32_t (&f)[4]) {
    const uint8_t *fbp = sbase + 16u * (size_t)vs_off(hh);
    const int32_t ln = vs_len(hh);
#pragma unroll
    for (int q = 0; q < 4; ++q) e[q] = dp[1 + q * G + g];
#pragma unroll
    for (int j = 0; j < 4; ++j) {
      const int32_t k = L * j + l;
      f[j] = k < ln ? *(const uint32_t *)(fbp + 4 * k) : 0u;
    }
  };
  uint64_t h1 = 0, h2 = 0;
  uint64_t e_cur[4] = {0, 0, 0, 0}, e_nxt[4] = {0, 0, 0, 0};
  uint32_t f_cur[4] = {0, 0, 0, 0}, f_nxt[4] = {0, 0, 0, 0};
  if (wave < nbatch) {
    h1 = dsc[0];
    load_batch(dsc, h1, e_cur, f_cur);
  }
  if (wave + NW < nbatch) h2 = dsc[(size_t)NW * W64];
  for (int32_t bi = wave; bi < nbatch; bi += NW) {
    uint64_t h3 = 0;
    if (bi + 2 * NW < nbatch) h3 = dsc[(size_t)2 * NW * W64];
    if (bi + NW < nbatch) load_batch(dsc + (size_t)NW * W64, h2, e_nxt, f_nxt);
    const int32_t len = vs_len(h1);
    const int cls = vs_cls(h1);
    int32_t row[4], sh[4];
#pragma unroll
    for (int q = 0; q < 4; ++q) {
      row[q] = (int32_t)(uint32_t)e_cur[q];
      sh[q] = (int32_t)(e_cur[q] >> 32);
    }
    double acc[4] = {0.0, 0.0, 0.0, 0.0};
#pragma unroll
    for (int j = 0; j < 4; ++j) {
// ... 76 lines not shown
```

fictitious_domain_al_preconditioners_amd/solver.py:

```python
from __future__ import annotations

import ctypes as C
import os

import numpy as np

from . import _abi

_HERE = os.path.dirname(os.path.abspath(__file__))
LIB_PATH = os.path.join(_HERE, "lib", "libalfd.so")
_lib = None

ABI_SYMBOLS = [
    "alfd_abi_version", "alfd_strerror", "alfd_last_error", "alfd_create", "alfd_destroy",
    "alfd_comm_unique_id", "alfd_comm_init", "alfd_set_partition", "alfd_set_matrix", "alfd_set_diag",
    "alfd_configure", "alfd_default_config", "alfd_setup", "alfd_precond_apply", "alfd_system_apply",
    "alfd_augment_rhs", "alfd_solve", "alfd_upload_rhs", "alfd_solve_resident", "alfd_download_solution",
    "alfd_get_history", "alfd_spmv", "alfd_dot", "alfd_matrix_lanes", "alfd_bench_spmv",
    "alfd_enable_timing", "alfd_get_timing", "alfd_host_halo_plan", "alfd_local_group_create",
    "alfd_local_group_destroy", "alfd_comm_init_local", "alfd_set_aggregates",
    "alfd_set_aggregate_partition", "alfd_get_matrix_info", "alfd_bench_spmv_format",
    "alfd_host_window_plan", "alfd_set_tunable", "alfd_build_aggregates", "alfd_get_aggregates",
    "alfd_host_aggregate_level", "alfd_comm_init_host",
    "alfd_get_device_memory", "alfd_set_row_blocks", "alfd_host_stream_plan",
    "alfd_host_row_blocks_from_points", "alfd_host_stream_plan_short", "alfd_set_prolongator", "alfd_set_controls", "alfd_get_timing_streamed", "alfd_get_setup_seconds",
    "alfd_host_numbering_from_points", "alfd_host_brick_blocks_from_points", "alfd_host_permute_csr",
    "alfd_build_smoothed_aggregation", "alfd_get_prolongator", "alfd_host_smoothed_prolongator",
    "alfd_inner_prec_apply",
]


class AlfdError(RuntimeError):

    def __init__(self, status, message):
        super().__init__(f"alfd status {status}: {message}")
        self.status = status


class NoConvergence(AlfdError):
    pass


def load_library():
    global _lib
    if _lib is not None:
        return _lib
    if not os.path.exists(LIB_PATH):
        raise ImportError(f"{LIB_PATH} is missing: the HIP extension is required (no CPU fallback). "
                          "Build it with `python -c 'import __graft_entry__ as g; g.build()'`.")
    lib = C.CDLL(LIB_PATH)
    vp, i32, i64, dbl = C.c_void_p, C.c_int32, C.c_int64, C.c_double
    PP = C.POINTER(C.c_void_p)
    sig = {
        "alfd_abi_version": (C.c_int, []),
        "alfd_strerror": (C.c_char_p, [C.c_int]),
        "alfd_last_error": (C.c_char_p, [vp]),
        "alfd_create": (C.c_int, [C.POINTER(vp), C.c_int]),
        "alfd_destroy": (C.c_int, [vp]),
        "alfd_comm_unique_id": (C.c_int, [vp, C.c_size_t]),
        "alfd_comm_init": (C.c_int, [vp, C.c_int, C.c_int, vp, C.c_size_t]),
        "alfd_set_partition": (C.c_int, [vp, C.c_int, PP]),
        "alfd_set_matrix": (C.c_int, [vp, C.c_int, i64, i64, vp, vp, vp]),
        "alfd_set_diag": (C.c_int, [vp, C.c_int, i64, vp]),
        "alfd_configure": (C.c_int, [vp, C.POINTER(_abi.Config)]),
        "alfd_default_config": (None, [C.POINTER(_abi.Config), C.c_int]),
        "alfd_setup": (C.c_int, [vp]),
        "alfd_precond_apply": (C.c_int, [vp, PP, PP, C.POINTER(_abi.Result)]),
        "alfd_system_apply": (C.c_int, [vp, PP, PP]),
        "alfd_augment_rhs": (C.c_int, [vp, PP]),
        "alfd_solve": (C.c_int, [vp, PP, PP, C.POINTER(_abi.Result)]),
        "alfd_upload_rhs": (C.c_int, [vp, PP, PP]),
        "alfd_solve_resident": (C.c_int, [vp, C.POINTER(_abi.Result)]),
        "alfd_download_solution": (C.c_int, [vp, PP]),
        "alfd_get_history": (C.c_int, [vp, vp, i32, C.POINTER(i32)]),
        "alfd_spmv": (C.c_int, [vp, C.c_int, vp, vp, C.c_int, dbl]),
        "alfd_dot": (C.c_int, [vp, i64, vp, vp, C.POINTER(dbl)]),
        "alfd_inner_prec_apply": (C.c_int, [vp, C.c_int, vp, vp]),
        "alfd_matrix_lanes": (C.c_int, [vp, C.c_int, C.POINTER(i32)]),
        "alfd_bench_spmv": (C.c_int, [vp, C.c_int, i32, C.POINTER(dbl), C.POINTER(dbl)]),
        "alfd_enable_timing": (C.c_int, [vp, C.c_int]),
        "alfd_get_timing": (C.c_int, [vp, vp, vp, vp]),
        "alfd_host_halo_plan": (C.c_int, [i64, vp, vp, C.c_int, C.c_int, vp, vp, i64, C.POINTER(i64), vp]),
        "alfd_local_group_create": (C.c_int, [C.c_int, C.POINTER(vp)]),
        "alfd_local_group_destroy": (C.c_int, [vp]),
        "alfd_comm_init_local": (C.c_int, [vp, vp, C.c_int]),
        "alfd_set_aggregates": (C.c_int, [vp, C.c_int, i64, vp, vp, i64]),
        "alfd_set_aggregate_partition": (C.c_int, [vp, C.c_int, vp]),
        "alfd_set_prolongator": (C.c_int, [vp, C.c_int, i64, i64, vp, vp, vp]),
        "alfd_set_controls": (C.c_int, [vp, vp, vp, vp]),
        "alfd_get_timing_streamed": (C.c_int, [vp, vp]),
        "alfd_get_setup_seconds": (C.c_int, [vp, vp]),
        "alfd_get_matrix_info": (C.c_int, [vp, C.c_int, C.POINTER(_abi.MatrixInfo)]),
        "alfd_bench_spmv_format": (C.c_int, [vp, C.c_int, i32, C.c_int, C.POINTER(dbl), C.POINTER(dbl)]),
        "alfd_host_window_plan": (C.c_int, [i64, vp, vp, vp, i32, i32, C.POINTER(_abi.WindowPlanInfo)]),
        "alfd_set_tunable": (C.c_int, [vp, C.c_char_p, C.c_int]),
        "alfd_build_aggregates": (C.c_int, [vp, i32, dbl, i32, i64, i32, C.POINTER(i32)]),
        "alfd_get_aggregates": (C.c_int, [vp, C.c_int, vp, i64, C.POINTER(i64), C.POINTER(i64)]),
        "alfd_host_aggregate_level": (C.c_int, [i64, vp, vp, vp, i32, dbl, i32, vp, C.POINTER(i64)]),
        "alfd_build_smoothed_aggregation": (C.c_int, [vp, i32, dbl, i32, dbl, i64, i32, C.POINTER(i32), vp]),
        "alfd_get_prolongator": (C.c_int, [vp, C.c_int, vp, vp, vp, i64, C.POINTER(i64), C.POINTER(i64),
                                           C.POINTER(i64)]),
        "alfd_host_smoothed_prolongator": (C.c_int, [i64, vp, vp, vp, i64, vp, vp, vp, vp, dbl, vp, i64, dbl,
                                                     vp, vp, vp, i64, C.POINTER(i64)]),
        "alfd_comm_init_host": (C.c_int, [vp, C.c_int, C.c_int, vp, vp, vp]),
        "alfd_get_device_memory": (C.c_int, [vp, C.POINTER(i64), C.POINTER(i64)]),
        "alfd_set_row_blocks": (C.c_int, [vp, C.c_int, i64, vp, vp]),
        "alfd_host_stream_plan": (C.c_int, [i64, vp, vp, vp, C.c_int32, i64, vp, vp, vp]),
        "alfd_host_row_blocks_from_points": (C.c_int, [i64, C.c_int32, vp, C.c_int32, vp, vp, vp]),
        "alfd_host_stream_plan_short": (C.c_int, [i64, vp, vp, vp, C.c_int32, vp]),
        "alfd_host_numbering_from_points": (C.c_int, [i64, C.c_int32, vp, vp]),
        "alfd_host_brick_blocks_from_points": (C.c_int, [i64, C.c_int32, vp, vp, C.c_int32, vp, vp, vp]),
        "alfd_host_permute_csr": (C.c_int, [i64, vp, vp, vp, vp, vp, vp, vp, vp]),
    }
    for name, (res, args) in sig.items():
        fn = getattr(lib, name)
        fn.restype = res
        fn.argtypes = args
    _lib = lib
    return lib


def _blocks(arrs):
    a = (C.c_void_p * len(arrs))()
    for i, x in enumerate(arrs):
        a[i] = x.ctypes.data
    return a


class Context:

    def __init__(self, device_id=0):
        self._lib = load_library()
        self._h = C.c_void_p()
        rc = self._lib.alfd_create(C.byref(self._h), device_id)
        if rc != _abi.OK:
            self._h = None
            raise AlfdError(rc, "alfd_create failed: " + self._lib.alfd_strerror(rc).decode() +
                            " (a HIP device is required; there is no CPU path)")
        self.block_sizes = None
        self.cfg = None

    def close(self):
        if getattr(self, "_h", None):
            self._lib.alfd_destroy(self._h)
            self._h = None

    __del__ = close

    def _ck(self, rc):
        if rc != _abi.OK:
            msg = self._lib.alfd_last_error(self._h).decode() or self._lib.alfd_strerror(rc).decode()
            cls = NoConvergence if rc in (_abi.E_NO_CONVERGENCE_OUTER, _abi.E_NO_CONVERGENCE_INNER) else AlfdError
            raise cls(rc, msg)

    @staticmethod
    def unique_id() -> bytes:
        buf = C.create_string_buffer(_abi.UNIQUE_ID_BYTES)
        rc = load_library().alfd_comm_unique_id(buf, _abi.UNIQUE_ID_BYTES)
        if rc != _abi.OK:
            raise AlfdError(rc, "alfd_comm_unique_id failed")
        return buf.raw

    def comm_init(self, rank, nranks, unique_id: bytes):
        self._ck(self._lib.alfd_comm_init(self._h, rank, nranks, unique_id, len(unique_id)))

    def comm_init_local(self, group, rank):
        self._ck(self._lib.alfd_comm_init_local(self._h, group, rank))

    def comm_init_torch(self, group=None):
        from . import hostcomm
        rank, world, ag, a2a = hostcomm.torch_callbacks(group)
        self._host_cbs = (ag, a2a)
        self._ck(self._lib.alfd_comm_init_host(self._h, rank, world, C.cast(ag, C.c_void_p), C.cast(a2a, C.c_void_p),
                                               None))
# ... 134 lines not shown

    def history(self):
        cnt = C.c_int32(0)
        self._lib.alfd_get_history(self._h, None, 0, C.byref(cnt))
        out = np.zeros(max(cnt.value, 1))
        self._lib.alfd_get_history(self._h, out.ctypes.data, cnt.value, C.byref(cnt))
        return out[:cnt.value]

    def spmv(self, slot, x, y=None, mode=0, alpha=1.0):
        x = np.ascontiguousarray(x, np.float64)
        lanes = C.c_int32()
        self._ck(self._lib.alfd_matrix_lanes(self._h, slot, C.byref(lanes)))
        if y is None:
            raise ValueError("pass y (its length is the row count)")
        y = np.ascontiguousarray(y, np.float64).copy()
        self._ck(self._lib.alfd_spmv(self._h, slot, x.ctypes.data, y.ctypes.data, mode, alpha))
        return y, lanes.value

    def dot(self, x, y):
        x = np.ascontiguousarray(x, np.float64)
        y = np.ascontiguousarray(y, np.float64)
        out = C.c_double()
        self._ck(self._lib.alfd_dot(self._h, x.size, x.ctypes.data, y.ctypes.data, C.byref(out)))
        return out.value

    def inner_prec_apply(self, r, op=_abi.INNER_OP_AUG):
        r = np.ascontiguousarray(r, np.float64)
        bs = self.block_sizes
        if bs is None:
            n = r.size
        else:
            n = {_abi.INNER_OP_AUG: bs[0], _abi.INNER_OP_A22: bs[1]}.get(op, bs[0] + bs[1])
            if r.size != n:
                raise ValueError(f"r has {r.size} entries, the inner operator {n}")
        z = np.zeros(n)
        self._ck(self._lib.alfd_inner_prec_apply(self._h, int(op), r.ctypes.data, z.ctypes.data))
        return z

    def bench_spmv(self, slot, reps=20):
        ms, nbytes = C.c_double(), C.c_double()
        self._ck(self._lib.alfd_bench_spmv(self._h, slot, reps, C.byref(ms), C.byref(nbytes)))
        return ms.value, nbytes.value

    def bench_spmv_format(self, slot, reps=20, value_index=True):
        ms, nbytes = C.c_double(), C.c_double()
        self._ck(self._lib.alfd_bench_spmv_format(self._h, slot, reps, int(value_index), C.byref(ms),
                                                  C.byref(nbytes)))
        return ms.value, nbytes.value

    def matrix_info(self, slot):
        info = _abi.MatrixInfo()
        self._ck(self._lib.alfd_get_matrix_info(self._h, slot, C.byref(info)))
        return {k: getattr(info, k) for k, _ in info._fields_ if k != "reserved"}

    def set_tunable(self, name, value):
        self._ck(self._lib.alfd_set_tunable(self._h, name.encode(), int(value)))

    def set_row_blocks(self, slot, block_ptr, rows):
        if block_ptr is None:
            self._ck(self._lib.alfd_set_row_blocks(self._h, slot, 0, None, None))
            return
        bp = np.ascontiguousarray(block_ptr, np.int64)
        rw = np.ascontiguousarray(rows, np.int32)
        self._ck(self._lib.alfd_set_row_blocks(self._h, slot, bp.size - 1, bp.ctypes.data, rw.ctypes.data))

    def device_memory(self):
        f, t = C.c_int64(0), C.c_int64(0)
        self._ck(self._lib.alfd_get_device_memory(self._h, C.byref(f), C.byref(t)))
        return f.value, t.value

    def enable_timing(self, on=True):
        self._ck(self._lib.alfd_enable_timing(self._h, int(on)))

    def timing(self):
        ms = np.zeros(_abi.T_NCLASSES)
        n = np.zeros(_abi.T_NCLASSES, np.int64)
        b = np.zeros(_abi.T_NCLASSES)
        self._ck(self._lib.alfd_get_timing(self._h, ms.ctypes.data, n.ctypes.data, b.ctypes.data))
        fb = np.zeros(_abi.T_NCLASSES)
        self._ck(self._lib.alfd_get_timing_streamed(self._h, fb.ctypes.data))
        names = ["spmv_A", "spmv_other", "dot", "vec"]
        return {k: dict(ms=float(ms[i]), launches=int(n[i]), bytes=float(b[i]), format_bytes=float(fb[i]))
                for i, k in enumerate(names)}

    def setup_seconds(self):
        s = np.zeros(8)
        self._ck(self._lib.alfd_get_setup_seconds(self._h, s.ctypes.data))
        names = ["upload", "diag_lambda", "ml_fetch", "ml_galerkin", "ml_upload", "ml_lambda", "ml_patch", "ml_coarse"]
        return {k: float(s[i]) for i, k in enumerate(names)}


class LocalGroup:

    def __init__(self, nranks):
        self._lib = load_library()
        self.handle = C.c_void_p()
        rc = self._lib.alfd_local_group_create(nranks, C.byref(self.handle))
        if rc != _abi.OK:
            raise AlfdError(rc, "alfd_local_group_create failed")
        self.nranks = nranks

    def close(self):
        if self.handle:
            self._lib.alfd_local_group_destroy(self.handle)
            self.handle = None


def host_halo_plan(col, col_offsets, rank):
    lib = load_library()
    col = np.ascontiguousarray(col, np.int32)
    offs = np.ascontiguousarray(col_offsets, np.int64)
    nranks = offs.size - 1
    col_local = np.empty_like(col)
    halo = np.empty(max(col.size, 1), np.int32)
    n_halo = C.c_int64()
    recv_off = np.zeros(nranks + 1, np.int64)
    rc = lib.alfd_host_halo_plan(col.size, col.ctypes.data, offs.ctypes.data, nranks, rank,
                                 col_local.ctypes.data, halo.ctypes.data, halo.size, C.byref(n_halo),
                                 recv_off.ctypes.data)
    if rc != _abi.OK:
        raise AlfdError(rc, "alfd_host_halo_plan failed")
    return col_local, halo[:n_halo.value].copy(), recv_off


def host_aggregate_level(m, block_size=1, threshold=0.02, max_aggregate_nodes=8):
    lib = load_library()
    rp = np.ascontiguousarray(m.row_ptr, np.int64)
    col = np.ascontiguousarray(m.col, np.int32)
    val = np.ascontiguousarray(m.val, np.float64)
    agg = np.empty(m.nrows, np.int32)
    nc = C.c_int64(0)
    rc = lib.alfd_host_aggregate_level(m.nrows, rp.ctypes.data, col.ctypes.data, val.ctypes.data, block_size,
                                       threshold, max_aggregate_nodes, agg.ctypes.data, C.byref(nc))
    if rc != _abi.OK:
        raise AlfdError(rc, "alfd_host_aggregate_level failed")
    return agg, int(nc.value)


def host_smoothed_prolongator(A, agg, n_coarse, omega, Ct=None, w_inv=None, gamma=0.0):
    from .problems import Csr
    lib = load_library()
    rp = np.ascontiguousarray(A.row_ptr, np.int64)
    col = np.ascontiguousarray(A.col, np.int32)
    val = np.ascontiguousarray(A.val, np.float64)
    agg = np.ascontiguousarray(agg, np.int32)
    if agg.size != A.nrows:
        raise ValueError("agg must have one entry per row of A")
    if Ct is not None:
        crp = np.ascontiguousarray(Ct.row_ptr, np.int64)
        ccol = np.ascontiguousarray(Ct.col, np.int32)
        cval = np.ascontiguousarray(Ct.val, np.float64)
        w = np.ascontiguousarray(w_inv, np.float64)
        if w.size != Ct.ncols:
            raise ValueError("w_inv must have one entry per column of Ct")
        pen = (int(Ct.ncols), crp.ctypes.data, ccol.ctypes.data, cval.ctypes.data, w.ctypes.data, float(gamma))
    else:
        pen = (0, None, None, None, None, 0.0)
    prp = np.empty(A.nrows + 1, np.int64)
    nnz = C.c_int64(0)

    def call(pc, pv, cap):
        return lib.alfd_host_smoothed_prolongator(A.nrows, rp.ctypes.data, col.ctypes.data, val.ctypes.data, *pen,
                                                  agg.ctypes.data, int(n_coarse), float(omega), prp.ctypes.data, pc,
                                                  pv, cap, C.byref(nnz))
    rc = call(None, None, 0)
    if rc != _abi.OK:
# ... 264 lines not shown
```

include/alfd/alfd.h:

```cpp
#ifndef ALFD_H
#define ALFD_H

#include <stddef.h>
#include <stdint.h>

#ifdef __cplusplus
extern "C" {
#endif

#define ALFD_ABI_VERSION 12
#define ALFD_MAX_BLOCKS 3

enum alfd_status {
  ALFD_OK = 0,
  ALFD_E_INVALID = 1,
  ALFD_E_HIP = 2,
  ALFD_E_NO_CONVERGENCE_OUTER = 3,
  ALFD_E_NO_CONVERGENCE_INNER = 4,
  ALFD_E_BREAKDOWN = 5,
  ALFD_E_NOT_SETUP = 6,
  ALFD_E_COMM = 7,
  ALFD_E_UNSUPPORTED = 8
};

// ... 142 lines not shown
                        int64_t *n_coarse);
int alfd_host_aggregate_level(int64_t nrows, const int64_t *row_ptr, const int32_t *col, const double *val,
                              int32_t block_size, double threshold, int32_t max_aggregate_nodes, int32_t *agg,
                              int64_t *n_coarse);
int alfd_build_smoothed_aggregation(alfd_ctx_t ctx, int32_t block_size, double threshold, int32_t max_aggregate_nodes,
                                    double damping, int64_t min_coarse, int32_t max_levels, int32_t *levels_out,
                                    double *omega_out);
int alfd_get_prolongator(alfd_ctx_t ctx, int level, int64_t *row_ptr, int32_t *col, double *val, int64_t capacity,
                         int64_t *n_fine, int64_t *n_coarse, int64_t *nnz);
int alfd_host_smoothed_prolongator(int64_t nrows, const int64_t *row_ptr, const int32_t *col, const double *val,
                                   int64_t n_mult, const int64_t *ct_row_ptr, const int32_t *ct_col, const double *ct_val,
                                   const double *w_inv, double gamma, const int32_t *agg, int64_t n_coarse, double omega,
                                   int64_t *p_row_ptr, int32_t *p_col, double *p_val, int64_t capacity, int64_t *nnz);
int alfd_configure(alfd_ctx_t ctx, const alfd_config *cfg);
int alfd_set_controls(alfd_ctx_t ctx, const alfd_control *outer, const alfd_control *inner, const alfd_control *mp_inner);
void alfd_default_config(alfd_config *cfg, int variant);
int alfd_setup(alfd_ctx_t ctx);

int alfd_precond_apply(alfd_ctx_t ctx, const double *const *src_blocks, double *const *dst_blocks,
                       alfd_result *res);
int alfd_system_apply(alfd_ctx_t ctx, const double *const *src_blocks, double *const *dst_blocks);
int alfd_augment_rhs(alfd_ctx_t ctx, double *const *rhs_blocks);
int alfd_solve(alfd_ctx_t ctx, const double *const *rhs_blocks, double *const *x_blocks,
               alfd_result *res);
int alfd_upload_rhs(alfd_ctx_t ctx, const double *const *rhs_blocks, const double *const *x0_blocks);
int alfd_solve_resident(alfd_ctx_t ctx, alfd_result *res);
int alfd_download_solution(alfd_ctx_t ctx, double *const *x_blocks);
int alfd_get_history(alfd_ctx_t ctx, double *out, int32_t capacity, int32_t *count);

int alfd_spmv(alfd_ctx_t ctx, int slot, const double *x, double *y, int mode, double alpha);
int alfd_dot(alfd_ctx_t ctx, int64_t n, const double *x, const double *y, double *result);
enum alfd_inner_op { ALFD_INNER_OP_AUG = 0, ALFD_INNER_OP_A22 = 1, ALFD_INNER_OP_AUG2 = 2 };
int alfd_inner_prec_apply(alfd_ctx_t ctx, int op, const double *r, double *z);
int alfd_matrix_lanes(alfd_ctx_t ctx, int slot, int32_t *lanes);
int alfd_bench_spmv(alfd_ctx_t ctx, int slot, int32_t reps, double *ms_per_launch,
                    double *algorithmic_bytes);
typedef struct alfd_matrix_info {
  int32_t lanes, windowed, value_indexed;
  int32_t batch_major;
  int64_t nnz, window_blocks, window_fallback_blocks;
  int64_t value_indexed_blocks, value_indexed_nnz, dictionary_entries, value_wide_nnz;
  double algorithmic_bytes, streamed_bytes;
  int64_t shared_nnz;
  int64_t batch_major_blocks;
  int64_t batch_major_wide;
  int64_t batch_major_interior_blocks;
} alfd_matrix_info;
int alfd_get_matrix_info(alfd_ctx_t ctx, int slot, alfd_matrix_info *out);
typedef struct alfd_window_plan_info {
  int32_t windowed, value_indexed, row_block, max_window;
  int64_t blocks, fallback_blocks, segments;
  int64_t value_indexed_blocks, value_indexed_nnz, value_wide_nnz, dictionary_entries;
  int64_t batches, decode_mismatches;
} alfd_window_plan_info;
int alfd_host_window_plan(int64_t nrows, const int64_t *row_ptr, const int32_t *col, const double *val,
                          int32_t lanes, int32_t want_value_index, alfd_window_plan_info *out);
typedef struct alfd_stream_plan_info {
  int32_t ok, max_window, max_rows, max_batches;
  int64_t blocks, batches, segments, dictionary_entries, stream_bytes;
  int64_t decode_mismatches, rows_covered;
  int64_t shared_nnz;
} alfd_stream_plan_info;
int alfd_host_stream_plan(int64_t nrows, const int64_t *row_ptr, const int32_t *col, const double *val,
                          int32_t row_block, int64_t n_blocks, const int64_t *block_ptr, const int32_t *rows,
                          alfd_stream_plan_info *out);
int alfd_host_stream_plan_short(int64_t nrows, const int64_t *row_ptr, const int32_t *col, const double *val,
                                int32_t lanes, alfd_stream_plan_info *out);
int alfd_bench_spmv_format(alfd_ctx_t ctx, int slot, int32_t reps, int use_value_index,
                           double *ms_per_launch, double *streamed_bytes);
int alfd_set_row_blocks(alfd_ctx_t ctx, int slot, int64_t n_blocks, const int64_t *block_ptr, const int32_t *rows);

int alfd_host_row_blocks_from_points(int64_t nrows, int32_t dim, const double *points, int32_t max_rows,
                                     int64_t *n_blocks_out, int64_t *block_ptr_out, int32_t *rows_out);

int alfd_host_numbering_from_points(int64_t nrows, int32_t dim, const double *points, int64_t *new_to_old);
int alfd_host_brick_blocks_from_points(int64_t nrows, int32_t dim, const double *points, const int32_t *brick,
                                       int32_t max_rows, int64_t *n_blocks_out, int64_t *block_ptr_out, int32_t *rows_out);
int alfd_host_permute_csr(int64_t nrows, const int64_t *row_ptr, const int32_t *col, const double *val,
                          const int64_t *row_new_to_old, const int64_t *col_old_to_new, int64_t *out_row_ptr,
                          int32_t *out_col, double *out_val);

int alfd_get_device_memory(alfd_ctx_t ctx, int64_t *free_bytes, int64_t *total_bytes);
int alfd_set_tunable(alfd_ctx_t ctx, const char *name, int value);
enum alfd_timing_class {
  ALFD_T_SPMV_A = 0,
  ALFD_T_SPMV_OTHER = 1,
  ALFD_T_DOT = 2,
  ALFD_T_VEC = 3,
  ALFD_T_NCLASSES = 4
};
int alfd_enable_timing(alfd_ctx_t ctx, int on);
int alfd_get_timing(alfd_ctx_t ctx, double *ms , int64_t *launches ,
                    double *algorithmic_bytes );
int alfd_get_timing_streamed(alfd_ctx_t ctx, double *streamed_bytes );
enum alfd_setup_phase {
  ALFD_SETUP_UPLOAD = 0,
  ALFD_SETUP_DIAG_LAMBDA = 1,
  ALFD_SETUP_ML_FETCH = 2,
  ALFD_SETUP_ML_GALERKIN = 3,
  ALFD_SETUP_ML_UPLOAD = 4,
  ALFD_SETUP_ML_LAMBDA = 5,
  ALFD_SETUP_ML_PATCH = 6,
  ALFD_SETUP_ML_COARSE = 7,
  ALFD_SETUP_NPHASES = 8
};
int alfd_get_setup_seconds(alfd_ctx_t ctx, double *seconds );

#ifdef __cplusplus
}
#endif
#endif
```

Baseline: 14.87.

## Fuse paired A and C SpMVs into one split-grid kernel launch

```diff
diff --git a/fictitious_domain_al_preconditioners_amd/_abi.py b/fictitious_domain_al_preconditioners_amd/_abi.py
--- a/fictitious_domain_al_preconditioners_amd/_abi.py
+++ b/fictitious_domain_al_preconditioners_amd/_abi.py
@@ -20,6 +20,10 @@
 INNER_THROW, INNER_ACCEPT = range(2)
 T_SPMV_A, T_SPMV_OTHER, T_DOT, T_VEC = range(4)
 T_NCLASSES = 4
+PAIR_NFIRST = 3
+PAIR_NSECOND = 6
+PAIR_FIRST_NAMES = ("batch_major", "stream", "plain")
+PAIR_SECOND_NAMES = ("plain4", "plain8", "plain16", "plain32", "plain64", "stream")
 UNIQUE_ID_BYTES = 128
 
 
diff --git a/fictitious_domain_al_preconditioners_amd/csrc/alfd.hip b/fictitious_domain_al_preconditioners_amd/csrc/alfd.hip
--- a/fictitious_domain_al_preconditioners_amd/csrc/alfd.hip
+++ b/fictitious_domain_al_preconditioners_amd/csrc/alfd.hip
@@ -235,6 +235,8 @@
   bool dots_replicated = false;
   int64_t ml_rep_threshold = 300000;
   int ml_fuse = 1;
+  int ml_pair = 1;
+  int64_t pair_count[ALFD_PAIR_NFIRST * ALFD_PAIR_NSECOND] = {};
   int ml_gpu_galerkin = 1;
   double *g_w = nullptr, *g_tlam = nullptr;
   std::vector<int64_t> ml_coff[ALFD_MAX_LEVELS];
@@ -660,9 +662,7 @@
 #undef ALFD_VSS
 }
 
-static bool launch_vs(alfd_ctx *ctx, const DevCsr &m, const double *x, double *y, int epi, double alpha,
-                      const double *d, double *y2, int64_t first_block = 0, int64_t n_blocks = -1) {
-  const DevCsr::Vs &v = m.vs;
+static bool vs_lds_base_ok(alfd_ctx *ctx) {
   if (ctx->vs_lds_base_ok < 0) {
     uint32_t *probe = nullptr, base = 1;
     if (hipMalloc((void **)&probe, sizeof(uint32_t)) == hipSuccess) {
@@ -675,7 +675,13 @@
     if (!ctx->vs_lds_base_ok)
       std::fprintf(stderr, "[alfd] dynamic LDS does not start at offset 0 (%u): batch-major SpMV formats disabled\n", base);
   }
-  if (!ctx->vs_lds_base_ok) return false;
+  return ctx->vs_lds_base_ok != 0;
+}
+
+static bool launch_vs(alfd_ctx *ctx, const DevCsr &m, const double *x, double *y, int epi, double alpha,
+                      const double *d, double *y2, int64_t first_block = 0, int64_t n_blocks = -1) {
+  const DevCsr::Vs &v = m.vs;
+  if (!vs_lds_base_ok(ctx)) return false;
   if (v.L == 32) return launch_vss<32>(ctx, m, x, y, epi, alpha, d, y2), true;
   if (v.L == 16) return launch_vss<16>(ctx, m, x, y, epi, alpha, d, y2), true;
   if (v.L == 8) return launch_vss<8>(ctx, m, x, y, epi, alpha, d, y2), true;
@@ -3411,9 +3417,75 @@
   return F;
 }
 
+
+static int pair_form(alfd_ctx *ctx, const DevCsr &m) {
+  if (m.vs.on && ctx->vs_enable && !ctx->vi_off && vs_lds_base_ok(ctx))
+    return m.vs.L == 64 && !m.vs.wide && m.tag != 0 ? ALFD_PAIR_BATCH_MAJOR : -1;
+  if (m.win) return -1;
+  if (m.L == 64 && !m.sparse && ctx->spmv_stream_R > 0)
+    return ctx->spmv_stream_R == 2 && ctx->spmv_stream_U == 8 && !ctx->spmv_nt ? ALFD_PAIR_STREAM : -1;
+  return m.L == 4 || m.L == 8 || m.L == 16 || m.L == 32 || m.L == 64 ? ALFD_PAIR_PLAIN : -1;
+}
+
+static unsigned pair_blocks(const alfd_ctx *ctx, const DevCsr &m, int form) {
+  if (form == ALFD_PAIR_BATCH_MAJOR) return (unsigned)m.vs.nb;
+  if (form == ALFD_PAIR_PLAIN) return (unsigned)grid_for_rows(m.n_list, m.L);
+  const int64_t nbatches = (m.nrows + 1) / 2;
+  return (unsigned)std::max<int64_t>(1, std::min<int64_t>((nbatches + 3) / 4, 256 * ctx->spmv_grid_mult));
+}
+
+static PairCsr pair_operand(const DevCsr &m, int form, double *y, const double *d) {
+  PairCsr p;
+  p.nrows = form == ALFD_PAIR_STREAM ? m.nrows : m.n_list;
+  p.rp = m.rp, p.col = m.col, p.val = m.val;
+  p.rows = m.sparse ? m.rows : nullptr;
+  p.x_halo = m.halo, p.n_local = m.n_local_cols;
+  p.form = form == ALFD_PAIR_STREAM ? 0 : m.L;
+  p.y = y, p.d = d;
+  return p;
+}
+
+static int spmv_pair(alfd_ctx *ctx, DevCsr &A, int clsA, DevCsr &C, const double *x, double *y, const double *w, double *tlam) {
+  int fa = -1, fc = -1;
+  if (ctx->ml_pair && ctx->nranks == 1 && clsA != ALFD_T_SPMV_A && A.present && C.present && A.n_list > 0 && C.n_list > 0) {
+    fa = pair_form(ctx, A);
+    fc = pair_form(ctx, C);
+  }
+  if (fa < 0 || fc < 0 || fc == ALFD_PAIR_BATCH_MAJOR) {
+    RC(spmv_m(ctx, A, clsA, x, y, 0));
+    return spmv_m(ctx, C, ALFD_T_SPMV_OTHER, x, tlam, 2, 0.0, w);
+  }
+  if (A.sparse) HIPC(hipMemsetAsync(y, 0, A.nrows * sizeof(double), ctx->stream));
+  if (C.sparse) HIPC(hipMemsetAsync(tlam, 0, C.nrows * sizeof(double), ctx->stream));
+  const bool use_vi = !ctx->vi_off, use_vs = ctx->vs_enable != 0 && !ctx->vi_off;
+  Timer tm(ctx, clsA, A.algorithmic_bytes() + C.algorithmic_bytes(), A.streamed_bytes(use_vi, use_vs) + C.streamed_bytes(use_vi, use_vs));
+  const unsigned n_first = pair_blocks(ctx, A, fa), n_second = pair_blocks(ctx, C, fc);
+  const unsigned grid = n_first + n_second;
+  const PairCsr pc = pair_operand(C, fc, tlam, w);
+  if (fa == ALFD_PAIR_BATCH_MAJOR) {
+    const DevCsr::Vs &v = A.vs;
+    PairVs pa;
+    pa.stream = v.stream, pa.tab = v.tab, pa.hdrb = v.hdrb, pa.segx = v.segx, pa.dict = v.dict, pa.x_halo = A.halo;
+    pa.y = y, pa.stride = v.stride, pa.seg_stride = v.seg_stride, pa.n_local = A.n_local_cols, pa.xcd_remap = ctx->vs_xcd;
+    const size_t lds = (size_t)VsFmt<0>::kWinOff + (size_t)v.maxW * sizeof(double);
+    hipLaunchKernelGGL(spmv_pair_vs_kernel, dim3(grid), dim3(256), lds, ctx->stream, pa, pc, x, n_first, n_second);
+  } else {
+    const PairCsr pa = pair_operand(A, fa, y, nullptr);
+    if (fa == ALFD_PAIR_STREAM)
+      hipLaunchKernelGGL(spmv_pair_kernel<0>, dim3(grid), dim3(kBlock), 0, ctx->stream, pa, pc, x, n_first, n_second);
+    else
+      hipLaunchKernelGGL(spmv_pair_kernel<1>, dim3(grid), dim3(kBlock), 0, ctx->stream, pa, pc, x, n_first, n_second);
+  }
+  HIPC(hipGetLastError());
+  const int second = fc == ALFD_PAIR_STREAM ? ALFD_PAIR_SECOND_STREAM
+                     : C.L == 4 ? ALFD_PAIR_SECOND_L4 : C.L == 8 ? ALFD_PAIR_SECOND_L8 : C.L == 16 ? ALFD_PAIR_SECOND_L16
+                     : C.L == 32 ? ALFD_PAIR_SECOND_L32 : ALFD_PAIR_SECOND_L64;
+  ctx->pair_count[fa * ALFD_PAIR_NSECOND + second]++;
+  return ALFD_OK;
+}
+
 static int fused_AC(alfd_ctx *ctx, const AugOp &F, const double *x, double *y) {
-  RC(spmv_m(ctx, *F.A, F.clsA, x, y, 0));
-  return spmv_m(ctx, *F.C, ALFD_T_SPMV_OTHER, x, F.tlam, 2, 0.0, F.w);
+  return spmv_pair(ctx, *F.A, F.clsA, *F.C, x, y, F.w, F.tlam);
 }
 
 static int aug_apply(alfd_ctx *ctx, const AugOp &F, const double *x, double *y) {
@@ -3636,15 +3708,13 @@
   }
   RC(ml_cycle(ctx, 0, Q.rr, z));
   hipLaunchKernelGGL(scatter_add_kernel, dim3(gm), dim3(256), 0, ctx->stream, Q.m, Q.S, Q.zS, z);
-  RC(spmv_m(ctx, Q.As, ALFD_T_SPMV_OTHER, z, Q.uS, 0));
-  if (fused_ok(ctx, F)) {
-    RC(spmv(ctx, ALFD_C, z, ctx->t_lam, 2, 0.0, w));
+  const bool fuse = fused_ok(ctx, F);
+  if (fuse || pen) RC(spmv_pair(ctx, Q.As, ALFD_T_SPMV_OTHER, ctx->mat[ALFD_C], z, Q.uS, w, ctx->t_lam));
+  else RC(spmv_m(ctx, Q.As, ALFD_T_SPMV_OTHER, z, Q.uS, 0));
+  if (fuse) {
     RC(fused_correct(ctx, F, pdeg, pratio, Q.rS, Q.uS, Q.eS, nullptr));
   } else {
-    if (pen) {
-      RC(spmv(ctx, ALFD_C, z, ctx->t_lam, 2, 0.0, w));
-      RC(spmv_m(ctx, Q.Cts, ALFD_T_SPMV_OTHER, ctx->t_lam, Q.uS, 1, ctx->cfg.gamma));
-    }
+    if (pen) RC(spmv_m(ctx, Q.Cts, ALFD_T_SPMV_OTHER, ctx->t_lam, Q.uS, 1, ctx->cfg.gamma));
     VEC_LAUNCH(sub_from_kernel, Q.mpad, 24, Q.rS, Q.uS);
     RC(aug_cheb(ctx, F, pdeg, pratio, Q.uS, Q.eS));
   }
@@ -5457,6 +5527,7 @@
   if (const char *e = std::getenv("ALFD_ML_REPLICATE")) ctx->ml_rep_threshold = std::atoll(e);
   if (const char *e = std::getenv("ALFD_ML_GPU_GALERKIN")) ctx->ml_gpu_galerkin = std::atoi(e);
   if (const char *e = std::getenv("ALFD_ML_FUSE")) ctx->ml_fuse = std::atoi(e) != 0;
+  if (const char *e = std::getenv("ALFD_ML_PAIR")) ctx->ml_pair = std::atoi(e) != 0;
   if (const char *e = std::getenv("ALFD_SPMV_VI_LEVELS")) ctx->vi_levels = std::atoi(e);
   if (const char *e = std::getenv("ALFD_SPMV_BATCH_MAJOR")) ctx->vs_enable = std::atoi(e);
   if (const char *e = std::getenv("ALFD_SPMV_BATCH_MAJOR_ROWS")) ctx->vs_RB = std::max(4, std::min(kVsMaxRows, std::atoi(e)));
@@ -6715,6 +6786,10 @@
     ctx->ml_fuse = value != 0;
     return ALFD_OK;
   }
+  if (std::strcmp(name, "ml_pair") == 0) {
+    ctx->ml_pair = value != 0;
+    return ALFD_OK;
+  }
   if (std::strcmp(name, "nested_mp_group") == 0) {
     if (value < 1 || value > 1000) return ctx->err = "nested_mp_group: 1..1000", ALFD_E_INVALID;
     ctx->nmp_group = value;
@@ -6758,6 +6833,12 @@
   return ALFD_OK;
 }
 
+int alfd_get_pair_counts(alfd_ctx_t ctx, int64_t *counts) {
+  if (!ctx || !counts) return ALFD_E_INVALID;
+  for (int i = 0; i < ALFD_PAIR_NFIRST * ALFD_PAIR_NSECOND; ++i) counts[i] = ctx->pair_count[i];
+  return ALFD_OK;
+}
+
 int alfd_get_timing(alfd_ctx_t ctx, double *ms, int64_t *launches, double *bytes) {
   if (!ctx) return ALFD_E_INVALID;
   flush_timers(ctx);
diff --git a/fictitious_domain_al_preconditioners_amd/csrc/kernels.hpp b/fictitious_domain_al_preconditioners_amd/csrc/kernels.hpp
--- a/fictitious_domain_al_preconditioners_amd/csrc/kernels.hpp
+++ b/fictitious_domain_al_preconditioners_amd/csrc/kernels.hpp
@@ -148,6 +148,53 @@
   return (lds4[0] + lds4[1]) + (lds4[2] + lds4[3]);
 }
 
+struct GridReal {
+  __device__ __forceinline__ uint32_t idx() const { return blockIdx.x; }
+  __device__ __forceinline__ uint32_t cnt() const { return gridDim.x; }
+};
+struct GridPart {
+  uint32_t vb, nvb;
+  __device__ __forceinline__ uint32_t idx() const { return vb; }
+  __device__ __forceinline__ uint32_t cnt() const { return nvb; }
+};
+template <int L, int EPI, int SPARSE, class G>
+__device__ __forceinline__ void spmv_body(const G &grid, int64_t nrows, const int64_t *__restrict__ rp,
+                                          const int32_t *__restrict__ col, const double *__restrict__ val,
+                                          const int32_t *__restrict__ rows, const double *__restrict__ x,
+                                          const double *__restrict__ x_halo, int32_t n_local, double *__restrict__ y,
+                                          double alpha, const double *__restrict__ d, double *__restrict__ y2) {
+  constexpr int RPB = kBlock / L;
+  const int lane = threadIdx.x % L;
+  const int sub = threadIdx.x / L;
+  const int64_t ngroups = (nrows + RPB - 1) / RPB;
+  for (int64_t g = grid.idx(); g < ngroups; g += grid.cnt()) {
+    const int64_t r = g * RPB + sub;
+    if (r < nrows) {
+      const int64_t k0 = rp[r], k1 = rp[r + 1];
+      double acc = 0.0;
+      for (int64_t k = k0 + lane; k < k1; k += L) {
+        const int32_t c = col[k];
+        const double xv = (c < n_local) ? x[c] : x_halo[c - n_local];
+        acc = fma(val[k], xv, acc);
+      }
+      acc = group_reduce<L>(acc);
+      if (lane == 0) {
+        const int64_t ro = (SPARSE == 2 ? rows != nullptr : SPARSE != 0) ? (int64_t)rows[r] : r;
+        if (EPI == 0)
+          y[ro] = acc;
+        else if (EPI == 1)
+          y[ro] = fma(alpha, acc, y[ro]);
+        else if (EPI == 2)
+          y[ro] = d[ro] * acc;
+        else {
+          y[ro] = acc;
+          y2[ro] = d[ro] * acc;
+        }
+      }
+    }
+  }
+}
+
 template <int L, int EPI, bool SPARSE>
 __global__ __launch_bounds__(kBlock) void spmv_kernel(int64_t nrows, const int64_t *__restrict__ rp,
                                                       const int32_t *__restrict__ col,
@@ -158,36 +205,7 @@
                                                       double *__restrict__ y, double alpha,
                                                       const double *__restrict__ d,
                                                       double *__restrict__ y2) {
-  constexpr int RPB = kBlock / L;
-  const int lane = threadIdx.x % L;
-  const int sub = threadIdx.x / L;
-  const int64_t ngroups = (nrows + RPB - 1) / RPB;
-  for (int64_t g = blockIdx.x; g < ngroups; g += gridDim.x) {
-    const int64_t r = g * RPB + sub;
-    if (r < nrows) {
-      const int64_t k0 = rp[r], k1 = rp[r + 1];
-      double acc = 0.0;
-      for (int64_t k = k0 + lane; k < k1; k += L) {
-        const int32_t c = col[k];
-        const double xv = (c < n_local) ? x[c] : x_halo[c - n_local];
-        acc = fma(val[k], xv, acc);
-      }
-      acc = group_reduce<L>(acc);
-      if (lane == 0) {
-        const int64_t ro = SPARSE ? (int64_t)rows[r] : r;
-        if (EPI == 0)
-          y[ro] = acc;
-        else if (EPI == 1)
-          y[ro] = fma(alpha, acc, y[ro]);
-        else if (EPI == 2)
-          y[ro] = d[ro] * acc;
-        else {
-          y[ro] = acc;
-          y2[ro] = d[ro] * acc;
-        }
-      }
-    }
-  }
+  spmv_body<L, EPI, SPARSE ? 1 : 0>(GridReal(), nrows, rp, col, val, rows, x, x_halo, n_local, y, alpha, d, y2);
 }
 
 template <int R, int U, int EPI, bool NT>
@@ -196,75 +214,83 @@
     const double *__restrict__ val, const double *__restrict__ x, const double *__restrict__ x_halo,
     int32_t n_local, double *__restrict__ y, double alpha, const double *__restrict__ d,
     double *__restrict__ y2) {
-  const int lane = threadIdx.x & 63;
-  const int wave = __builtin_amdgcn_readfirstlane(threadIdx.x >> 6);
-  const int64_t nbatches = (nrows + R - 1) / R;
-  for (int64_t b = (int64_t)blockIdx.x * 4 + wave; b < nbatches; b += (int64_t)gridDim.x * 4) {
-    const int64_t r0 = b * R;
-    int64_t kb[R + 1];
-#pragma unroll
-    for (int i = 0; i <= R; ++i) kb[i] = rp[r0 + i < nrows ? r0 + i : nrows];
-    const int64_t k_begin = kb[0];
-    const int32_t n_batch = (int32_t)(kb[R] - k_begin);
-    int32_t rel[R + 1];
-#pragma unroll
-    for (int i = 0; i <= R; ++i) rel[i] = (int32_t)(kb[i] - k_begin);
-    double acc[R];
-#pragma unroll
-    for (int i = 0; i < R; ++i) acc[i] = 0.0;
-    const int32_t *cb = col + k_begin;
-    const double *vb = val + k_begin;
-    for (int32_t base = 0; base < n_batch; base += 64 * U) {
-      int32_t c[U];
-      double v[U], xv[U];
-#pragma unroll
-      for (int u = 0; u < U; ++u) {
-        const int32_t o = base + 64 * u + lane;
-        if (o < n_batch) {
-          c[u] = NT ? __builtin_nontemporal_load(cb + o) : cb[o];
-          v[u] = NT ? __builtin_nontemporal_load(vb + o) : vb[o];
-        } else {
-          c[u] = -1;
-          v[u] = 0.0;
-        }
-      }
-#pragma unroll
-      for (int u = 0; u < U; ++u) {
-        xv[u] = 0.0;
-        if (c[u] >= 0) xv[u] = (c[u] < n_local) ? x[c[u]] : x_halo[c[u] - n_local];
-      }
-#pragma unroll
-      for (int u = 0; u < U; ++u) {
-        const int32_t o = base + 64 * u + lane;
-        if (c[u] >= 0) {
-#pragma unroll
-          for (int i = 0; i < R; ++i)
-            if (o >= rel[i] && o < rel[i + 1]) acc[i] = fma(v[u], xv[u], acc[i]);
-        }
-      }
-    }
-#pragma unroll
-    for (int i = 0; i < R; ++i) {
-      const int64_t r = r0 + i;
-      if (r < nrows) {
-        const int dsh = rel[i] & 63;
-        double s = __shfl(acc[i], (lane + dsh) & 63, 64);
-        s = group_reduce<64>(s);
-        if (lane == 0) {
-          if (EPI == 0)
-            y[r] = s;
-          else if (EPI == 1)
-            y[r] = fma(alpha, s, y[r]);
-          else if (EPI == 2)
-            y[r] = d[r] * s;
-          else {
-            y[r] = s;
-            y2[r] = d[r] * s;
-          }
-        }
-      }
-    }
-  }
+#define ALFD_BLOCK_IDX blockIdx.x
+#define ALFD_BLOCK_CNT gridDim.x
+#include "kernels_stream_body.inc"
+#undef ALFD_BLOCK_IDX
+#undef ALFD_BLOCK_CNT
+}
+
+template <int R, int U, int EPI, bool NT>
+__device__ __forceinline__ void spmv_stream_body(
+    const GridPart &grid,
+    int64_t nrows, const int64_t *__restrict__ rp, const int32_t *__restrict__ col,
+    const double *__restrict__ val, const double *__restrict__ x, const double *__restrict__ x_halo,
+    int32_t n_local, double *__restrict__ y, double alpha, const double *__restrict__ d,
+    double *__restrict__ y2) {
+#define ALFD_BLOCK_IDX grid.vb
+#define ALFD_BLOCK_CNT grid.nvb
+#include "kernels_stream_body.inc"
+#undef ALFD_BLOCK_IDX
+#undef ALFD_BLOCK_CNT
+}
+
+struct PairCsr {
+  int64_t nrows;
+  const int64_t *rp;
+  const int32_t *col;
+  const double *val;
+  const int32_t *rows;
+  const double *x_halo;
+  int32_t n_local;
+  int32_t form;
+  double *y;
+  const double *d;
+};
+
+template <int U>
+__device__ __forceinline__ void spmv_pair_second(const GridPart &g, const PairCsr &c, const double *__restrict__ x) {
+#define ALFD_SECOND(LL) \
+  spmv_body<LL, 2, 2>(g, c.nrows, c.rp, c.col, c.val, c.rows, x, c.x_halo, c.n_local, c.y, 0.0, c.d, nullptr)
+  switch (c.form) {
+    case 0: spmv_stream_body<2, U, 2, false>(g, c.nrows, c.rp, c.col, c.val, x, c.x_halo, c.n_local, c.y, 0.0, c.d, nullptr); break;
+    case 4: ALFD_SECOND(4); break;
+    case 8: ALFD_SECOND(8); break;
+    case 16: ALFD_SECOND(16); break;
+    case 32: ALFD_SECOND(32); break;
+    default: ALFD_SECOND(64); break;
+  }
+#undef ALFD_SECOND
+}
+
+__device__ __forceinline__ bool spmv_pair_split(uint32_t n_first, uint32_t n_second, GridPart &g) {
+  const uint32_t b = blockIdx.x;
+  if (b < n_first) return g.vb = b, g.nvb = n_first, false;
+  return g.vb = b - n_first, g.nvb = n_second, true;
+}
+
+template <int FIRST>
+__global__ __launch_bounds__(kBlock) void spmv_pair_kernel(PairCsr a, PairCsr c, const double *__restrict__ x,
+                                                           uint32_t n_first, uint32_t n_second) {
+  GridPart g;
+  if (spmv_pair_split(n_first, n_second, g)) {
+    spmv_pair_second<8>(g, c, x);
+    return;
+  }
+  if (FIRST == 0) {
+    spmv_stream_body<2, 8, 0, false>(g, a.nrows, a.rp, a.col, a.val, x, a.x_halo, a.n_local, a.y, 0.0, nullptr, nullptr);
+    return;
+  }
+#define ALFD_FIRST(LL) \
+  spmv_body<LL, 0, 2>(g, a.nrows, a.rp, a.col, a.val, a.rows, x, a.x_halo, a.n_local, a.y, 0.0, nullptr, nullptr)
+  switch (a.form) {
+    case 4: ALFD_FIRST(4); break;
+    case 8: ALFD_FIRST(8); break;
+    case 16: ALFD_FIRST(16); break;
+    case 32: ALFD_FIRST(32); break;
+    default: ALFD_FIRST(64); break;
+  }
+#undef ALFD_FIRST
 }
 
 template <int R, int U, int EPI, int TAG = 0>
diff --git a/fictitious_domain_al_preconditioners_amd/csrc/kernels_stream_body.inc b/fictitious_domain_al_preconditioners_amd/csrc/kernels_stream_body.inc
--- /dev/null
+++ b/fictitious_domain_al_preconditioners_amd/csrc/kernels_stream_body.inc
@@ -0,0 +1,69 @@
+  const int lane = threadIdx.x & 63;
+  const int wave = __builtin_amdgcn_readfirstlane(threadIdx.x >> 6);
+  const int64_t nbatches = (nrows + R - 1) / R;
+  for (int64_t b = (int64_t)ALFD_BLOCK_IDX * 4 + wave; b < nbatches; b += (int64_t)ALFD_BLOCK_CNT * 4) {
+    const int64_t r0 = b * R;
+    int64_t kb[R + 1];
+#pragma unroll
+    for (int i = 0; i <= R; ++i) kb[i] = rp[r0 + i < nrows ? r0 + i : nrows];
+    const int64_t k_begin = kb[0];
+    const int32_t n_batch = (int32_t)(kb[R] - k_begin);
+    int32_t rel[R + 1];
+#pragma unroll
+    for (int i = 0; i <= R; ++i) rel[i] = (int32_t)(kb[i] - k_begin);
+    double acc[R];
+#pragma unroll
+    for (int i = 0; i < R; ++i) acc[i] = 0.0;
+    const int32_t *cb = col + k_begin;
+    const double *vb = val + k_begin;
+    for (int32_t base = 0; base < n_batch; base += 64 * U) {
+      int32_t c[U];
+      double v[U], xv[U];
+#pragma unroll
+      for (int u = 0; u < U; ++u) {
+        const int32_t o = base + 64 * u + lane;
+        if (o < n_batch) {
+          c[u] = NT ? __builtin_nontemporal_load(cb + o) : cb[o];
+          v[u] = NT ? __builtin_nontemporal_load(vb + o) : vb[o];
+        } else {
+          c[u] = -1;
+          v[u] = 0.0;
+        }
+      }
+#pragma unroll
+      for (int u = 0; u < U; ++u) {
+        xv[u] = 0.0;
+        if (c[u] >= 0) xv[u] = (c[u] < n_local) ? x[c[u]] : x_halo[c[u] - n_local];
+      }
+#pragma unroll
+      for (int u = 0; u < U; ++u) {
+        const int32_t o = base + 64 * u + lane;
+        if (c[u] >= 0) {
+#pragma unroll
+          for (int i = 0; i < R; ++i)
+            if (o >= rel[i] && o < rel[i + 1]) acc[i] = fma(v[u], xv[u], acc[i]);
+        }
+      }
+    }
+#pragma unroll
+    for (int i = 0; i < R; ++i) {
+      const int64_t r = r0 + i;
+      if (r < nrows) {
+        const int dsh = rel[i] & 63;
+        double s = __shfl(acc[i], (lane + dsh) & 63, 64);
+        s = group_reduce<64>(s);
+        if (lane == 0) {
+          if (EPI == 0)
+            y[r] = s;
+          else if (EPI == 1)
+            y[r] = fma(alpha, s, y[r]);
+          else if (EPI == 2)
+            y[r] = d[r] * s;
+          else {
+            y[r] = s;
+            y2[r] = d[r] * s;
+          }
+        }
+      }
+    }
+  }
diff --git a/fictitious_domain_al_preconditioners_amd/csrc/kernels_vs.hpp b/fictitious_domain_al_preconditioners_amd/csrc/kernels_vs.hpp
--- a/fictitious_domain_al_preconditioners_amd/csrc/kernels_vs.hpp
+++ b/fictitious_domain_al_preconditioners_amd/csrc/kernels_vs.hpp
@@ -119,176 +119,43 @@
     const double *__restrict__ dict, const double *__restrict__ x, const double *__restrict__ x_halo,
     int32_t n_local, double *__restrict__ y, double alpha, const double *__restrict__ d, double *__restrict__ y2,
     int xcd_remap, int32_t block_base) {
-  extern __shared__ double xs[];
-  char *sm = (char *)xs;
-  double *ds = (double *)(sm + kVsDictOff);
-  double *xw = (double *)(sm + VsFmt<WD>::kWinOff);
-  const int lane = threadIdx.x & 63;
-  const int wave = __builtin_amdgcn_readfirstlane(threadIdx.x >> 6);
-  int64_t b = blockIdx.x;
-  if (xcd_remap) {
-    const int64_t nwg = gridDim.x, q = nwg / 8, rm = nwg % 8, xcd = b % 8, idx = b / 8;
-    b = (xcd < rm ? xcd * (q + 1) : rm * (q + 1) + (xcd - rm) * q) + idx;
-  }
-  b += block_base;
-  const int32_t *hb = hdrb + 8 * b;
-  const int32_t nbatch = hb[0], W = hb[1], nseg = hb[2], nd = hb[3], doff = hb[4];
-  const uint8_t *sbase = stream + (int64_t)(((uint64_t)(uint32_t)hb[6] << 32) | (uint64_t)(uint32_t)hb[5]);
-  const int32_t *sx = segx + 2 * b * (int64_t)seg_stride;
-  const uint32_t *tb = (const uint32_t *)(tab + (int64_t)b * stride * 16);
-  const int hl = lane & 31;
-  auto hdr_at = [&](int32_t q) {
-    uint32_t h4 = 4u * (uint32_t)hl;
-    asm volatile("" : "+v"(h4));
-    return *(const uint32_t *)((const char *)(tb + 32 * (int64_t)q) + h4);
-  };
-  auto hdr_load = [&](int32_t q) {
-    return hdr_at(q < nbatch ? q : (nbatch > 0 ? nbatch - 1 : 0));
-  };
-  auto hdr = [](uint32_t hv, int k) { return (uint32_t)__builtin_amdgcn_readlane((int)hv, k); };
-  uint32_t hv1 = hdr_at(wave);
-  uint32_t hv2 = hdr_at(wave + NW);
-  uint32_t w[6];
-  {
-    constexpr int U = 4;
-    auto stage = [&](int32_t s) {
-      int32_t c0[U], o0[U], sl[U];
-      double v[U];
-#pragma unroll
-      for (int u = 0; u < U; ++u) {
-        const int32_t q = s + u;
-        c0[u] = sx[2 * q];
-        o0[u] = sx[2 * q + 1];
-        const int32_t on = sx[2 * q + 3];
-        sl[u] = q < nseg ? ((q + 1 < nseg ? on : W) - o0[u]) : 0;
-      }
-#pragma unroll
-      for (int u = 0; u < U; ++u) {
-        const int32_t c = c0[u] + (lane < sl[u] ? lane : 0);
-        v[u] = (c < n_local) ? x[c] : x_halo[c - n_local];
-      }
-#pragma unroll
-      for (int u = 0; u < U; ++u)
-        if (lane < sl[u]) xw[o0[u] + lane] = v[u];
-    };
-    for (int t = threadIdx.x; t < nd; t += 64 * NW) ds[t] = dict[doff + t];
-    if (wave < nbatch && (int32_t)hdr(hv1, 1) < 0) vs_shared_fetch(hdr(hv1, 0), sbase, lane, w);
-    stage(wave * U);
-    for (int32_t s = (wave + NW) * U; s < nseg; s += NW * U) stage(s);
-  }
-  __syncthreads();
-  const int q16 = lane >> 4;
-  const int rsel = 4 * (2 * ((((q16 & 1) << 1) | (q16 >> 1)) + 4 * ((lane >> 3) & 1) + 8 * ((lane >> 2) & 1)) + 1);
-  auto store = [&](double s, int32_t r, bool mine) {
-    if (mine && r >= 0) {
-      if (EPI == 0)
-        y[r] = s;
-      else if (EPI == 1)
-        y[r] = fma(alpha, s, y[r]);
-      else if (EPI == 2)
-        y[r] = d[r] * s;
-      else {
-        y[r] = s;
-        y2[r] = d[r] * s;
-      }
-    }
-  };
-  for (int32_t bi = wave; bi < nbatch; bi += NW) {
-    uint32_t lo[16];
-#pragma unroll
-    for (int i = 0; i < 16; ++i) lo[i] = hdr(hv1, 2 * i);
-    const bool shared = (int32_t)hdr(hv1, 1) < 0;
-    const bool sixteen = shared && (int32_t)hdr(hv1, 17) >= 0;
-    const bool eight = shared && !sixteen && (int32_t)hdr(hv1, 9) >= 0;
-    const uint32_t eb = vs_off(lo[0]);
-    const int cls = vs_cls(lo[0]);
-    const int32_t full = cls > 0 ? 64 * (cls - 1) : 0;
-    const uint8_t *fb = sbase + 16u * (size_t)eb;
-    double sres;
-    int mstep;
-    uint32_t n0, n1;
-    if (sixteen) {
-      const int32_t rem = vs_len(lo[0]) - full;
-      int32_t sh[16];
-      sh[0] = 0;
-#pragma unroll
-      for (int i = 1; i < 16; ++i) sh[i] = (int32_t)lo[i];
-      double acc[16] = {0.0, 0.0, 0.0, 0.0, 0.0, 0.0, 0.0, 0.0, 0.0, 0.0, 0.0, 0.0, 0.0, 0.0, 0.0, 0.0};
-      switch (cls) {
-        case 1: vs_shared<1, 16, WD>(rem, sh, lane, w, acc); break;
-        case 2: vs_shared<2, 16, WD>(rem, sh, lane, w, acc); break;
-        case 3: vs_shared<3, 16, WD>(rem, sh, lane, w, acc); break;
-        case 4: vs_shared<4, 16, WD>(rem, sh, lane, w, acc); break;
-        case 5: vs_shared<5, 16, WD>(rem, sh, lane, w, acc); break;
-        default: vs_shared<6, 16, WD>(rem, sh, lane, w, acc); break;
-      }
-      sres = reduce_rows16(acc, lane);
-      mstep = 4;
-    } else if (eight) {
-      const int32_t rem = vs_len(lo[0]) - full;
-      int32_t sh[8];
-      sh[0] = 0;
-#pragma unroll
-      for (int i = 1; i < 8; ++i) sh[i] = (int32_t)lo[i];
-      double acc[8] = {0.0, 0.0, 0.0, 0.0, 0.0, 0.0, 0.0, 0.0};
-      switch (cls) {
-        case 1: vs_shared<1, 8, WD>(rem, sh, lane, w, acc); break;
-        case 2: vs_shared<2, 8, WD>(rem, sh, lane, w, acc); break;
-        case 3: vs_shared<3, 8, WD>(rem, sh, lane, w, acc); break;
-        case 4: vs_shared<4, 8, WD>(rem, sh, lane, w, acc); break;
-        case 5: vs_shared<5, 8, WD>(rem, sh, lane, w, acc); break;
-        default: vs_shared<6, 8, WD>(rem, sh, lane, w, acc); break;
-      }
-      sres = reduce_rows8(acc[0], acc[1], acc[2], acc[3], acc[4], acc[5], acc[6], acc[7], lane);
-      mstep = 8;
-    } else if (shared) {
-      double acc[4] = {0.0, 0.0, 0.0, 0.0};
-      const int32_t rem = vs_len(lo[0]) - full;
-      const int32_t sh[4] = {0, (int32_t)lo[1], (int32_t)lo[2], (int32_t)lo[3]};
-      switch (cls) {
-        case 1: vs_shared<1, 4, WD>(rem, sh, lane, w, acc); break;
-        case 2: vs_shared<2, 4, WD>(rem, sh, lane, w, acc); break;
-        case 3: vs_shared<3, 4, WD>(rem, sh, lane, w, acc); break;
-        case 4: vs_shared<4, 4, WD>(rem, sh, lane, w, acc); break;
-        case 5: vs_shared<5, 4, WD>(rem, sh, lane, w, acc); break;
-        default: vs_shared<6, 4, WD>(rem, sh, lane, w, acc); break;
-      }
-      sres = reduce_rows4(acc[0], acc[1], acc[2], acc[3]);
-      mstep = 16;
-    } else {
-      double acc[4] = {0.0, 0.0, 0.0, 0.0};
-      int32_t rem[4], maxrem = 1;
-#pragma unroll
-      for (int i = 0; i < 4; ++i) {
-        rem[i] = vs_len(lo[i]) - full;
-        maxrem = rem[i] > maxrem ? rem[i] : maxrem;
-      }
-      switch (cls) {
-        case 1: vs_batch<1, WD>(rem, maxrem, lane, fb, sm, acc); break;
-        case 2: vs_batch<2, WD>(rem, maxrem, lane, fb, sm, acc); break;
-        case 3: vs_batch<3, WD>(rem, maxrem, lane, fb, sm, acc); break;
-        case 4: vs_batch<4, WD>(rem, maxrem, lane, fb, sm, acc); break;
-        case 5: vs_batch<5, WD>(rem, maxrem, lane, fb, sm, acc); break;
-        case 6: vs_batch<6, WD>(rem, maxrem, lane, fb, sm, acc); break;
-        default: break;
-      }
-      n0 = hdr(hv2, 0);
-      n1 = hdr(hv2, 1);
-      store(reduce_rows4(acc[0], acc[1], acc[2], acc[3]), (int32_t)__builtin_amdgcn_ds_bpermute(rsel, (int)hv1), (lane & 15) == 0);
-      mstep = 0;
-    }
-    int32_t rid = -1;
-    if (mstep) {
-      rid = (int32_t)((uint32_t)__builtin_amdgcn_ds_bpermute(rsel, (int)hv1) &
-                      (lane < 8 ? 0x7fffffffu : 0xffffffffu));
-      n0 = hdr(hv2, 0);
-      n1 = hdr(hv2, 1);
-    }
-    hv1 = hv2;
-    if (bi + NW < nbatch && (int32_t)n1 < 0) vs_shared_fetch(n0, sbase, lane, w);
-    hv2 = hdr_load(bi + 2 * NW);
-    if (mstep) store(sres, rid, (lane & (mstep - 1)) == 0);
-  }
+#define ALFD_BLOCK_IDX blockIdx.x
+#define ALFD_BLOCK_CNT gridDim.x
+#include "kernels_vs_body.inc"
+#undef ALFD_BLOCK_IDX
+#undef ALFD_BLOCK_CNT
+}
+
+struct PairVs {
+  const uint8_t *stream;
+  const uint64_t *tab;
+  const int32_t *hdrb, *segx;
+  const double *dict, *x_halo;
+  double *y;
+  int32_t stride, seg_stride, n_local, xcd_remap;
+};
+
+__global__ __launch_bounds__(256) __attribute__((amdgpu_waves_per_eu(8, 8))) void spmv_pair_vs_kernel(
+    PairVs a, PairCsr c, const double *__restrict__ x, uint32_t n_first, uint32_t n_second) {
+  GridPart g;
+  if (spmv_pair_split(n_first, n_second, g)) {
+    spmv_pair_second<4>(g, c, x);
+    return;
+  }
+  constexpr int EPI = 0, NW = 4, WD = 0;
+  const uint8_t *__restrict__ stream = a.stream;
+  const uint64_t *__restrict__ tab = a.tab;
+  const int32_t *__restrict__ hdrb = a.hdrb, *__restrict__ segx = a.segx;
+  const double *__restrict__ dict = a.dict, *__restrict__ x_halo = a.x_halo;
+  double *__restrict__ y = a.y, *y2 = nullptr;
+  const double alpha = 0.0, *d = nullptr;
+  const int32_t stride = a.stride, seg_stride = a.seg_stride, n_local = a.n_local, block_base = 0;
+  const int xcd_remap = a.xcd_remap;
+#define ALFD_BLOCK_IDX g.vb
+#define ALFD_BLOCK_CNT g.nvb
+#include "kernels_vs_body.inc"
+#undef ALFD_BLOCK_IDX
+#undef ALFD_BLOCK_CNT
 }
 
 template <int L, int EPI, int TAG>
diff --git a/fictitious_domain_al_preconditioners_amd/csrc/kernels_vs_body.inc b/fictitious_domain_al_preconditioners_amd/csrc/kernels_vs_body.inc
--- /dev/null
+++ b/fictitious_domain_al_preconditioners_amd/csrc/kernels_vs_body.inc
@@ -0,0 +1,170 @@
+  extern __shared__ double xs[];
+  char *sm = (char *)xs;
+  double *ds = (double *)(sm + kVsDictOff);
+  double *xw = (double *)(sm + VsFmt<WD>::kWinOff);
+  const int lane = threadIdx.x & 63;
+  const int wave = __builtin_amdgcn_readfirstlane(threadIdx.x >> 6);
+  int64_t b = ALFD_BLOCK_IDX;
+  if (xcd_remap) {
+    const int64_t nwg = ALFD_BLOCK_CNT, q = nwg / 8, rm = nwg % 8, xcd = b % 8, idx = b / 8;
+    b = (xcd < rm ? xcd * (q + 1) : rm * (q + 1) + (xcd - rm) * q) + idx;
+  }
+  b += block_base;
+  const int32_t *hb = hdrb + 8 * b;
+  const int32_t nbatch = hb[0], W = hb[1], nseg = hb[2], nd = hb[3], doff = hb[4];
+  const uint8_t *sbase = stream + (int64_t)(((uint64_t)(uint32_t)hb[6] << 32) | (uint64_t)(uint32_t)hb[5]);
+  const int32_t *sx = segx + 2 * b * (int64_t)seg_stride;
+  const uint32_t *tb = (const uint32_t *)(tab + (int64_t)b * stride * 16);
+  const int hl = lane & 31;
+  auto hdr_at = [&](int32_t q) {
+    uint32_t h4 = 4u * (uint32_t)hl;
+    asm volatile("" : "+v"(h4));
+    return *(const uint32_t *)((const char *)(tb + 32 * (int64_t)q) + h4);
+  };
+  auto hdr_load = [&](int32_t q) {
+    return hdr_at(q < nbatch ? q : (nbatch > 0 ? nbatch - 1 : 0));
+  };
+  auto hdr = [](uint32_t hv, int k) { return (uint32_t)__builtin_amdgcn_readlane((int)hv, k); };
+  uint32_t hv1 = hdr_at(wave);
+  uint32_t hv2 = hdr_at(wave + NW);
+  uint32_t w[6];
+  {
+    constexpr int U = 4;
+    auto stage = [&](int32_t s) {
+      int32_t c0[U], o0[U], sl[U];
+      double v[U];
+#pragma unroll
+      for (int u = 0; u < U; ++u) {
+        const int32_t q = s + u;
+        c0[u] = sx[2 * q];
+        o0[u] = sx[2 * q + 1];
+        const int32_t on = sx[2 * q + 3];
+        sl[u] = q < nseg ? ((q + 1 < nseg ? on : W) - o0[u]) : 0;
+      }
+#pragma unroll
+      for (int u = 0; u < U; ++u) {
+        const int32_t c = c0[u] + (lane < sl[u] ? lane : 0);
+        v[u] = (c < n_local) ? x[c] : x_halo[c - n_local];
+      }
+#pragma unroll
+      for (int u = 0; u < U; ++u)
+        if (lane < sl[u]) xw[o0[u] + lane] = v[u];
+    };
+    for (int t = threadIdx.x; t < nd; t += 64 * NW) ds[t] = dict[doff + t];
+    if (wave < nbatch && (int32_t)hdr(hv1, 1) < 0) vs_shared_fetch(hdr(hv1, 0), sbase, lane, w);
+    stage(wave * U);
+    for (int32_t s = (wave + NW) * U; s < nseg; s += NW * U) stage(s);
+  }
+  __syncthreads();
+  const int q16 = lane >> 4;
+  const int rsel = 4 * (2 * ((((q16 & 1) << 1) | (q16 >> 1)) + 4 * ((lane >> 3) & 1) + 8 * ((lane >> 2) & 1)) + 1);
+  auto store = [&](double s, int32_t r, bool mine) {
+    if (mine && r >= 0) {
+      if (EPI == 0)
+        y[r] = s;
+      else if (EPI == 1)
+        y[r] = fma(alpha, s, y[r]);
+      else if (EPI == 2)
+        y[r] = d[r] * s;
+      else {
+        y[r] = s;
+        y2[r] = d[r] * s;
+      }
+    }
+  };
+  for (int32_t bi = wave; bi < nbatch; bi += NW) {
+    uint32_t lo[16];
+#pragma unroll
+    for (int i = 0; i < 16; ++i) lo[i] = hdr(hv1, 2 * i);
+    const bool shared = (int32_t)hdr(hv1, 1) < 0;
+    const bool sixteen = shared && (int32_t)hdr(hv1, 17) >= 0;
+    const bool eight = shared && !sixteen && (int32_t)hdr(hv1, 9) >= 0;
+    const uint32_t eb = vs_off(lo[0]);
+    const int cls = vs_cls(lo[0]);
+    const int32_t full = cls > 0 ? 64 * (cls - 1) : 0;
+    const uint8_t *fb = sbase + 16u * (size_t)eb;
+    double sres;
+    int mstep;
+    uint32_t n0, n1;
+    if (sixteen) {
+      const int32_t rem = vs_len(lo[0]) - full;
+      int32_t sh[16];
+      sh[0] = 0;
+#pragma unroll
+      for (int i = 1; i < 16; ++i) sh[i] = (int32_t)lo[i];
+      double acc[16] = {0.0, 0.0, 0.0, 0.0, 0.0, 0.0, 0.0, 0.0, 0.0, 0.0, 0.0, 0.0, 0.0, 0.0, 0.0, 0.0};
+      switch (cls) {
+        case 1: vs_shared<1, 16, WD>(rem, sh, lane, w, acc); break;
+        case 2: vs_shared<2, 16, WD>(rem, sh, lane, w, acc); break;
+        case 3: vs_shared<3, 16, WD>(rem, sh, lane, w, acc); break;
+        case 4: vs_shared<4, 16, WD>(rem, sh, lane, w, acc); break;
+        case 5: vs_shared<5, 16, WD>(rem, sh, lane, w, acc); break;
+        default: vs_shared<6, 16, WD>(rem, sh, lane, w, acc); break;
+      }
+      sres = reduce_rows16(acc, lane);
+      mstep = 4;
+    } else if (eight) {
+      const int32_t rem = vs_len(lo[0]) - full;
+      int32_t sh[8];
+      sh[0] = 0;
+#pragma unroll
+      for (int i = 1; i < 8; ++i) sh[i] = (int32_t)lo[i];
+      double acc[8] = {0.0, 0.0, 0.0, 0.0, 0.0, 0.0, 0.0, 0.0};
+      switch (cls) {
+        case 1: vs_shared<1, 8, WD>(rem, sh, lane, w, acc); break;
+        case 2: vs_shared<2, 8, WD>(rem, sh, lane, w, acc); break;
+        case 3: vs_shared<3, 8, WD>(rem, sh, lane, w, acc); break;
+        case 4: vs_shared<4, 8, WD>(rem, sh, lane, w, acc); break;
+        case 5: vs_shared<5, 8, WD>(rem, sh, lane, w, acc); break;
+        default: vs_shared<6, 8, WD>(rem, sh, lane, w, acc); break;
+      }
+      sres = reduce_rows8(acc[0], acc[1], acc[2], acc[3], acc[4], acc[5], acc[6], acc[7], lane);
+      mstep = 8;
+    } else if (shared) {
+      double acc[4] = {0.0, 0.0, 0.0, 0.0};
+      const int32_t rem = vs_len(lo[0]) - full;
+      const int32_t sh[4] = {0, (int32_t)lo[1], (int32_t)lo[2], (int32_t)lo[3]};
+      switch (cls) {
+        case 1: vs_shared<1, 4, WD>(rem, sh, lane, w, acc); break;
+        case 2: vs_shared<2, 4, WD>(rem, sh, lane, w, acc); break;
+        case 3: vs_shared<3, 4, WD>(rem, sh, lane, w, acc); break;
+        case 4: vs_shared<4, 4, WD>(rem, sh, lane, w, acc); break;
+        case 5: vs_shared<5, 4, WD>(rem, sh, lane, w, acc); break;
+        default: vs_shared<6, 4, WD>(rem, sh, lane, w, acc); break;
+      }
+      sres = reduce_rows4(acc[0], acc[1], acc[2], acc[3]);
+      mstep = 16;
+    } else {
+      double acc[4] = {0.0, 0.0, 0.0, 0.0};
+      int32_t rem[4], maxrem = 1;
+#pragma unroll
+      for (int i = 0; i < 4; ++i) {
+        rem[i] = vs_len(lo[i]) - full;
+        maxrem = rem[i] > maxrem ? rem[i] : maxrem;
+      }
+      switch (cls) {
+        case 1: vs_batch<1, WD>(rem, maxrem, lane, fb, sm, acc); break;
+        case 2: vs_batch<2, WD>(rem, maxrem, lane, fb, sm, acc); break;
+        case 3: vs_batch<3, WD>(rem, maxrem, lane, fb, sm, acc); break;
+        case 4: vs_batch<4, WD>(rem, maxrem, lane, fb, sm, acc); break;
+        case 5: vs_batch<5, WD>(rem, maxrem, lane, fb, sm, acc); break;
+        case 6: vs_batch<6, WD>(rem, maxrem, lane, fb, sm, acc); break;
+        default: break;
+      }
+      n0 = hdr(hv2, 0);
+      n1 = hdr(hv2, 1);
+      store(reduce_rows4(acc[0], acc[1], acc[2], acc[3]), (int32_t)__builtin_amdgcn_ds_bpermute(rsel, (int)hv1), (lane & 15) == 0);
+      mstep = 0;
+    }
+    int32_t rid = -1;
+    if (mstep) {
+      rid = (int32_t)((uint32_t)__builtin_amdgcn_ds_bpermute(rsel, (int)hv1) &
+                      (lane < 8 ? 0x7fffffffu : 0xffffffffu));
+      n0 = hdr(hv2, 0);
+      n1 = hdr(hv2, 1);
+    }
+    hv1 = hv2;
+    if (bi + NW < nbatch && (int32_t)n1 < 0) vs_shared_fetch(n0, sbase, lane, w);
+    hv2 = hdr_load(bi + 2 * NW);
+    if (mstep) store(sres, rid, (lane & (mstep - 1)) == 0);
+  }
diff --git a/fictitious_domain_al_preconditioners_amd/solver.py b/fictitious_domain_al_preconditioners_amd/solver.py
--- a/fictitious_domain_al_preconditioners_amd/solver.py
+++ b/fictitious_domain_al_preconditioners_amd/solver.py
@@ -26,7 +26,7 @@
     "alfd_host_row_blocks_from_points", "alfd_host_stream_plan_short", "alfd_set_prolongator", "alfd_set_controls", "alfd_get_timing_streamed", "alfd_get_setup_seconds",
     "alfd_host_numbering_from_points", "alfd_host_brick_blocks_from_points", "alfd_host_permute_csr",
     "alfd_build_smoothed_aggregation", "alfd_get_prolongator", "alfd_host_smoothed_prolongator",
-    "alfd_inner_prec_apply",
+    "alfd_inner_prec_apply", "alfd_get_pair_counts",
 ]
 
 
@@ -90,6 +90,7 @@
         "alfd_set_controls": (C.c_int, [vp, vp, vp, vp]),
         "alfd_get_timing_streamed": (C.c_int, [vp, vp]),
         "alfd_get_setup_seconds": (C.c_int, [vp, vp]),
+        "alfd_get_pair_counts": (C.c_int, [vp, vp]),
         "alfd_get_matrix_info": (C.c_int, [vp, C.c_int, C.POINTER(_abi.MatrixInfo)]),
         "alfd_bench_spmv_format": (C.c_int, [vp, C.c_int, i32, C.c_int, C.POINTER(dbl), C.POINTER(dbl)]),
         "alfd_host_window_plan": (C.c_int, [i64, vp, vp, vp, i32, i32, C.POINTER(_abi.WindowPlanInfo)]),
@@ -390,6 +391,17 @@
         names = ["spmv_A", "spmv_other", "dot", "vec"]
         return {k: dict(ms=float(ms[i]), launches=int(n[i]), bytes=float(b[i]), format_bytes=float(fb[i]))
                 for i, k in enumerate(names)}
+
+    def pair_counts(self):
+        n = np.zeros((_abi.PAIR_NFIRST, _abi.PAIR_NSECOND), np.int64)
+        self._ck(self._lib.alfd_get_pair_counts(self._h, n.ctypes.data))
+        first, second = _abi.PAIR_FIRST_NAMES, _abi.PAIR_SECOND_NAMES
+        return {"first": {k: int(n[i].sum()) for i, k in enumerate(first)},
+                "second": {"plain": int(n[:, :5].sum()), "stream": int(n[:, 5].sum())},
+                "second_plain_lanes": {4 << j: int(n[:, j].sum()) for j in range(5)},
+                "pairs": {(first[i], second[j]): int(n[i, j]) for i in range(len(first)) for j in range(len(second))
+                          if n[i, j]},
+                "total": int(n.sum())}
 
     def setup_seconds(self):
         s = np.zeros(8)
diff --git a/include/alfd/alfd.h b/include/alfd/alfd.h
--- a/include/alfd/alfd.h
+++ b/include/alfd/alfd.h
@@ -248,6 +248,22 @@
 
 int alfd_get_device_memory(alfd_ctx_t ctx, int64_t *free_bytes, int64_t *total_bytes);
 int alfd_set_tunable(alfd_ctx_t ctx, const char *name, int value);
+enum alfd_pair_first {
+  ALFD_PAIR_BATCH_MAJOR = 0,
+  ALFD_PAIR_STREAM = 1,
+  ALFD_PAIR_PLAIN = 2,
+  ALFD_PAIR_NFIRST = 3
+};
+enum alfd_pair_second {
+  ALFD_PAIR_SECOND_L4 = 0,
+  ALFD_PAIR_SECOND_L8 = 1,
+  ALFD_PAIR_SECOND_L16 = 2,
+  ALFD_PAIR_SECOND_L32 = 3,
+  ALFD_PAIR_SECOND_L64 = 4,
+  ALFD_PAIR_SECOND_STREAM = 5,
+  ALFD_PAIR_NSECOND = 6
+};
+int alfd_get_pair_counts(alfd_ctx_t ctx, int64_t *counts );
 enum alfd_timing_class {
   ALFD_T_SPMV_A = 0,
   ALFD_T_SPMV_OTHER = 1,
```

Result: faster. 15.51, median of 6 (+4.3%).
